# raynbowy23/RegT-GCN

Measured on NVIDIA B200. Metric: regt_gcn_fwd_bwd_samples_per_s, higher is better.
Workload: dtype f32 (3xTF32 on the tensor cores: fp32-equivalent, 1e-5 parity)

## Files before the change

### regt-gcn_b200/csrc/api.cu

```cuda
#include <stdlib.h>

#include "common.cuh"

namespace regt {

constexpr int F = REGT_F;

Route route_of(const regt_args* a) {
  const char* e = getenv("REGT_UNFUSED");
  const bool unfused = e && e[0] == '1';
  const bool tf32x3 = a->precision == REGT_PREC_TF32X3, bf16 = a->precision == REGT_PREC_BF16;
  const bool fused_step = a->fuse_head && a->y && a->d_out && a->loss;
  Route r{};
  r.cell = bf16 ? CellPath::Bf16
                : !tf32x3 ? CellPath::Fp32 : (!unfused && cell_f_fits(a)) ? CellPath::Tf32x3Fused : CellPath::Tf32x3Unfused;
  if (bf16 && fused_step && head_tc_fits(a->H, a->O))
    r.head = HeadPath::Bf16;
  else if (tf32x3 && a->H % 32 == 0 && head_f_fits(a->O) && (long long)a->B * a->N >= 128 && a->out)
    r.head = HeadPath::Tf32x3;
  else if (fused_step && head_fused_fits(a->H, a->O))
    r.head = HeadPath::FusedFfma;
  else
    r.head = HeadPath::Rows;
  r.g_tiled = r.cell == CellPath::Tf32x3Fused || r.cell == CellPath::Bf16;
  r.hid_partials = r.cell == CellPath::Bf16 && (r.head == HeadPath::Bf16 || r.head == HeadPath::FusedFfma);
  return r;
}

Layout make_layout(const regt_args* a, void* base) {
  Layout L{};
  L.route = route_of(a);
  Carver c(base);
  const size_t H = a->H, T = a->T, R = a->plan.R > 0 ? a->plan.R : 1, O = a->O;
  const size_t BN = (size_t)a->B * a->N, rows = BN * T;
  const size_t nseg = a->plan.nseg;
  L.Wzr = c.take<float>((F + H) * 2 * H);
  L.Wc = c.take<float>((F + H) * H);
  L.czr = c.take<float>(2 * H);
  L.cc = c.take<float>(H);
  L.M0t = c.take<float>(F * H);
  L.M1t = c.take<float>(R * F * H);
  L.c0 = c.take<float>(H);
  L.Lsum = c.take<float>(H * H);
  L.probs = c.take<float>(T);
  L.S = c.take<float>(BN * F * T);
  L.U = c.take<float>((size_t)a->B * (nseg ? nseg : 1) * F * T);
  if (L.route.cell == CellPath::Tf32x3Fused) {
    const size_t nqt = (BN + 127) / 128, rowsP = T * nqt * 128;
    const bool inf = a->inference != 0;
    L.tc_img_f = c.take<unsigned char>(F_IMG_BYTES);
    L.tc_img_b = c.take<unsigned char>(F_IMG_BYTES);
    L.Zp = c.take<float>(inf ? (size_t)TC_MAX_CTAS * 128 * H : rowsP * H);
    L.Rp = c.take<float>(inf ? 4 : rowsP * H);
    L.Hcp = c.take<float>(inf ? 4 : rowsP * H);
    L.Xt = c.take<float>(BN * F * T);
    L.h = c.take<float>(inf ? 4 : rowsP * H);
    L.hR = c.take<float>(inf ? 4 : rowsP * H);
    L.D = c.take<float>(inf ? 4 : rowsP * 4 * H);
    L.Feat = c.take<float>(inf ? 4 : nqt * 128 * 32);
    L.FeatT = c.take<float>(inf ? 4 : rowsP * 32);
    L.tc_dpp = c.take<float>(2 * (T * TC_MAX_CTAS + 64));
  } else if (L.route.cell != CellPath::Bf16) {
    L.h = c.take<float>(rows * H);
    L.Z = c.take<float>(rows * H);
    L.Rg = c.take<float>(rows * H);
    L.Hc = c.take<float>(rows * H);
    L.hR = c.take<float>(rows * H);
    L.Hn = c.take<float>(rows * H);
    L.D = c.take<float>(rows * 4 * H);
    L.Feat = c.take<float>(a->precision == REGT_PREC_TF32X3 ? rows * 32 : 4);
    L.bsplit = c.take<float>(a->precision == REGT_PREC_TF32X3 ? gemm_nt_scratch_floats((int)H, 2 * (int)H) : 4);
  } else {
    const size_t nqt = (BN + 127) / 128, plane = T * nqt * 128 * H;
    L.tc_img_f = c.take<unsigned char>(TC_IMG_BYTES);
    L.tc_img_b = c.take<unsigned char>(TC_IMG_BYTES);
    L.Zp = c.take<float>(plane);
    L.Rp = c.take<float>(plane);
    L.Hcp = c.take<float>(plane);
    L.dhp_p = c.take<float>(a->mode == REGT_MODE_REGIONAL ? plane : 4);
    L.Xt = c.take<float>(BN * F * T);
    L.hid_part = c.take<float>(T * nqt * 128 * H);
    L.tc_wpart = c.take<float>((size_t)TC_MAX_CTAS * 128 * 192);
    L.tc_dpp = c.take<float>(T * TC_MAX_CTAS + 64);
  }
  if (a->precision == REGT_PREC_TF32X3) {
    L.hf_rh = c.take<float>(BN * H);
    L.hf_do32 = c.take<float>(BN * 32);
    L.hf_split = c.take<float>(max(gemm_nt_scratch_floats(HEAD_HID, (int)H), gemm_nt_scratch_floats((int)H, HEAD_HID)));
    L.hf_loss_floats = BN / 8 + 2;
    L.hf_loss = c.take<float>(L.hf_loss_floats);
  }
  L.a1 = c.take<float>(BN * HEAD_HID);
  L.G = c.take<float>(((BN + 127) / 128) * 128 * H);
  L.d_a1 = c.take<float>(BN * HEAD_HID);
  L.dB = c.take<float>(3 * H * H);
  L.dP = c.take<float>(3 * H * F);
  L.dcg = c.take<float>(3 * H);
  L.dM0 = c.take<float>(H * F);
  L.dM1 = c.take<float>(R * H * F);
  L.dc0 = c.take<float>(H);
  L.dprobs = c.take<float>(T);
  size_t pf = (size_t)3 * WGRAD_SPLITS * H * H;
  pf = max(pf, (size_t)WGRAD_SPLITS * 4 * H * 32);
  pf = max(pf, (size_t)3 * H * H + 2 * 1024 * 64);
  pf = max(pf, (size_t)WGRAD_SPLITS * (3 * H * H + 4 * H * 32));
  pf = max(pf, (size_t)(2048 + R + 2) * H * F);
  pf = max(pf, (size_t)128 * T);
  pf = max(pf, (size_t)128 * (O * HEAD_HID + HEAD_HID * H));
  pf = max(pf, (size_t)152 * HEAD_HID * (H + 32));
  pf = max(pf, BN / 64 + 2);
  pf += H * HEAD_HID + HEAD_HID * O + 64;
  L.hpart = c.take<float>((size_t)148 * (HEAD_HID * H + O * HEAD_HID + HEAD_HID + O + 8));
  L.part = c.take<float>(pf);
  L.part_floats = pf;
  L.m1cp = c.take<int32_t>(R + 2);
  L.total = align_up(c.off, 256);
  return L;
}

static int validate(const regt_args* a, const char* who) {
  REGT_CHECK(a != nullptr, "%s: args is NULL", who);
  REGT_CHECK(a->B > 0 && a->N > 0 && a->T > 0 && a->O > 0, "%s: bad dims B=%d N=%d T=%d O=%d", who, a->B, a->N, a->T, a->O);
  REGT_CHECK(a->H >= 8 && a->H % 8 == 0 && a->H <= 1024, "%s: H=%d must be a multiple of 8 in [8,1024]", who, a->H);
  REGT_CHECK(a->mode >= 0 && a->mode <= 2, "%s: bad mode %d", who, a->mode);
  REGT_CHECK(a->x_rows == 0 || a->x_rows >= a->N, "%s: x_rows=%d must be 0 or >= N=%d", who, a->x_rows, a->N);
  REGT_CHECK(a->plan.N == a->N, "%s: plan built for %d nodes, args say %d", who, a->plan.N, a->N);
  REGT_CHECK((long long)a->B * a->N * a->T < (1ll << 31), "%s: B*N*T overflows int32 rows", who);
  REGT_CHECK(a->workspace && a->workspace_bytes >= regt_workspace_bytes(a), "%s: workspace missing or too small", who);
  REGT_CHECK(a->precision >= 0 && a->precision <= 2, "%s: bad precision %d", who, a->precision);
  return 0;
}

}

using namespace regt;

extern "C" size_t regt_workspace_bytes(const regt_args* a) {
  if (!a) return 0;
  return make_layout(a, nullptr).total;
}

extern "C" int regt_cell_forward(const regt_args* a) {
  if (validate(a, "regt_cell_forward")) return -1;
  REGT_CHECK(a->x && a->out_hidden, "regt_cell_forward: x / out_hidden is NULL");
  if (a->precision == REGT_PREC_TF32X3)
    REGT_CHECK(a->H % 32 == 0, "precision tf32x3 needs hidden %% 32 == 0 (got %d); use precision fp32", a->H);
  Layout L = make_layout(a, a->workspace);
  cudaStream_t st = (cudaStream_t)a->stream;
  prof_mark("<begin>", st);
  switch (L.route.cell) {
    case CellPath::Fp32: return cell_forward_fp32(a, L, st);
    case CellPath::Tf32x3Unfused: return cell_forward_g(a, L, st);
    case CellPath::Tf32x3Fused: return cell_forward_f(a, L, st);
    case CellPath::Bf16: return cell_forward_tc(a, L, st);
  }
  return -1;
}

extern "C" int regt_cell_backward(const regt_args* a) {
  if (validate(a, "regt_cell_backward")) return -1;
  REGT_CHECK(!a->inference, "regt_cell_backward: the forward ran with inference=1 (no activations were saved)");
  if (a->precision == REGT_PREC_TF32X3)
    REGT_CHECK(a->H % 32 == 0, "precision tf32x3 needs hidden %% 32 == 0 (got %d); use precision fp32", a->H);
  Layout L = make_layout(a, a->workspace);
  cudaStream_t st = (cudaStream_t)a->stream;
  prof_mark("<begin>", st);
  switch (L.route.cell) {
    case CellPath::Fp32: return cell_backward_fp32(a, L, st);
    case CellPath::Tf32x3Unfused: return cell_backward_g(a, L, st);
    case CellPath::Tf32x3Fused: return cell_backward_f(a, L, st);
    case CellPath::Bf16: return cell_backward_tc(a, L, st);
  }
  return -1;
}

static int validate_x(const regt_args* a, const regt_xgrad_plan* xp, const char* who) {
  REGT_CHECK(a != nullptr, "%s: args is NULL", who);
  REGT_CHECK(a->precision != REGT_PREC_BF16, "%s: precision bf16 keeps no gate-gradient plane; use fp32 or tf32x3", who);
  REGT_CHECK(a->x_rows == 0 || a->x_rows == a->N,
             "%s: region shards (x_rows=%d != N=%d) are not supported: their halo rows belong to other ranks", who, a->x_rows, a->N);
  REGT_CHECK(!a->inference, "%s: the forward ran with inference=1 (no activations were saved)", who);
  if (validate(a, who)) return -1;
  REGT_CHECK(xp && xp->N == a->N && xp->n_src == 2 * a->N + a->plan.nseg && xp->rowptr && xp->col && xp->val,
             "%s: transposed plan missing or built for another graph", who);
  return 0;
}

extern "C" size_t regt_cell_backward_x_scratch_bytes(const regt_args* a, const regt_xgrad_plan* xp) {
  if (!a || !xp) return 0;
  return cell_backward_x_scratch_bytes(a, xp);
}

extern "C" int regt_cell_backward_x(const regt_args* a, const regt_xgrad_plan* xp, float* d_x, void* scratch,
                                    size_t scratch_bytes) {
  if (validate_x(a, xp, "regt_cell_backward_x")) return -1;
  REGT_CHECK(d_x, "regt_cell_backward_x: d_x is NULL");
  REGT_CHECK(scratch && scratch_bytes >= cell_backward_x_scratch_bytes(a, xp), "regt_cell_backward_x: scratch missing or too small");
  if (a->precision == REGT_PREC_TF32X3)
    REGT_CHECK(a->H % 32 == 0, "precision tf32x3 needs hidden %% 32 == 0 (got %d); use precision fp32", a->H);
  Layout L = make_layout(a, a->workspace);
  cudaStream_t st = (cudaStream_t)a->stream;
  prof_mark("<begin>", st);
  return cell_backward_x(a, L, xp, d_x, scratch, st);
}

extern "C" int regt_head_forward(const regt_args* a) {
  if (validate(a, "regt_head_forward")) return -1;
  REGT_CHECK(a->out_hidden && a->out, "regt_head_forward: out_hidden / out is NULL");
  Layout L = make_layout(a, a->workspace);
  prof_mark("<begin>", (cudaStream_t)a->stream);
  return head_forward(a, L, (cudaStream_t)a->stream);
}

extern "C" int regt_head_backward(const regt_args* a) {
  if (validate(a, "regt_head_backward")) return -1;
  REGT_CHECK(!a->inference, "regt_head_backward: the forward ran with inference=1 (no activations were saved)");
  Layout L = make_layout(a, a->workspace);
  prof_mark("<begin>", (cudaStream_t)a->stream);
  return head_backward(a, L, (cudaStream_t)a->stream);
}

extern "C" int regt_debug_route(const regt_args* a, int32_t* out) {
  REGT_CHECK(a && out, "regt_debug_route: args and out must be non-NULL");
  const Route r = route_of(a);
  out[0] = (int32_t)r.cell;
  out[1] = (int32_t)r.head;
  out[2] = r.g_tiled;
  out[3] = r.hid_partials;
  return 0;
}
```

### regt-gcn_b200/csrc/common.cuh

```cuda
#pragma once
#include <cuda_runtime.h>
#include <stdint.h>
#include <stdio.h>

#include "regt_b200.h"

namespace regt {

void set_error(const char* fmt, ...);
void count_launch(int n = 1);
void prof_mark(const char* name, cudaStream_t st);
cudaStream_t fork_side(cudaStream_t main);
int join_side(cudaStream_t main);

#define REGT_CHECK(cond, ...)         \
  do {                                \
    if (!(cond)) {                    \
      regt::set_error(__VA_ARGS__);   \
      return -1;                      \
    }                                 \
  } while (0)

#define REGT_CUDA(expr)                                                                  \
  do {                                                                                   \
    cudaError_t _e = (expr);                                                             \
    if (_e != cudaSuccess) {                                                             \
      regt::set_error("%s failed: %s (%s:%d)", #expr, cudaGetErrorString(_e), __FILE__, __LINE__); \
      return -2;                                                                         \
    }                                                                                    \
  } while (0)

#define REGT_LAUNCH_CHECK()                                                              \
  do {                                                                                   \
    regt::count_launch();                                                                \
    cudaError_t _e = cudaGetLastError();                                                 \
    if (_e != cudaSuccess) {                                                             \
      regt::set_error("kernel launch failed: %s (%s:%d)", cudaGetErrorString(_e), __FILE__, __LINE__); \
      return -3;                                                                         \
    }                                                                                    \
  } while (0)

#define REGT_LAUNCHED(name, st)       \
  do {                                \
    REGT_LAUNCH_CHECK();              \
    regt::prof_mark(name, st);        \
  } while (0)

inline size_t align_up(size_t v, size_t a) { return (v + a - 1) / a * a; }
inline int cdiv(long long a, long long b) { return (int)((a + b - 1) / b); }

struct Carver {
  char* base;
  size_t off;
  explicit Carver(void* p) : base((char*)p), off(0) {}
  template <typename T>
  T* take(size_t n) {
    off = align_up(off, 256);
    T* r = base ? (T*)(base + off) : (T*)nullptr;
    off += n * sizeof(T);
    return r;
  }
};

__device__ __forceinline__ float sigmoidf_(float v) { return 1.0f / (1.0f + expf(-v)); }

__device__ __forceinline__ size_t g_off(long long q, int n, int H, int tiled) {
  return tiled ? ((((size_t)(q >> 7) * (H >> 2) + (n >> 2)) * 128 + (size_t)(q & 127)) * 4 + (n & 3)) : ((size_t)q * H + n);
}

inline int sm_count() {
  static int n = 0;
  if (n == 0) {
    int dev = 0;
    if (cudaGetDevice(&dev) != cudaSuccess || cudaDeviceGetAttribute(&n, cudaDevAttrMultiProcessorCount, dev) != cudaSuccess || n <= 0) n = 148;
  }
  return n;
}

enum class CellPath { Fp32, Tf32x3Unfused, Tf32x3Fused, Bf16 };
enum class HeadPath { Rows, FusedFfma, Tf32x3, Bf16 };
struct Route {
  CellPath cell;
  HeadPath head;
  bool g_tiled;
  bool hid_partials;
};
Route route_of(const regt_args* a);
bool cell_f_fits(const regt_args* a);
bool head_fused_fits(int H, int O);
bool head_tc_fits(int H, int O);
bool head_f_fits(int O);

struct Layout {
  Route route;
  float* Wzr;
  float* Wc;
  float* czr;
  float* cc;
  float* M0t;
  float* M1t;
  float* c0;
  float* Lsum;
  float* probs;
  float* S;
  float* U;
  float* h;
  float* Z;
  float* Rg;
  float* Hc;
  float* hR;
  float* Hn;
  float* a1;
  float* G;
  float* d_a1;
  float* D;
  float* Feat;
  float* hf_rh;
  float* hf_do32;
  float* hf_split;
  float* hf_loss;
  size_t hf_loss_floats;
  float* FeatT;
  float* bsplit;
  float* dB;
  float* dP;
  float* dcg;
  float* dM0;
  float* dM1;
  float* dc0;
  float* dprobs;
  float* hpart;
  float* part;
  size_t part_floats;
  int32_t* m1cp;
  unsigned char* tc_img_f;
  unsigned char* tc_img_b;
  float *Zp, *Rp, *Hcp, *dhp_p;
  float* Xt;
  float* hid_part;
  float* tc_wpart;
  float* tc_dpp;
  size_t total;
};
constexpr int TC_MAX_CTAS = 160;
constexpr int TC_IMG_BYTES = 160 * 1024;
constexpr int F_IMG_BYTES = 432 * 1024;

Layout make_layout(const regt_args* a, void* base);

constexpr int HEAD_HID = 128;
constexpr int WGRAD_SPLITS = 64;

int cell_forward_fp32(const regt_args* a, const Layout& L, cudaStream_t st);
int cell_backward_fp32(const regt_args* a, const Layout& L, cudaStream_t st);
int cell_forward_g(const regt_args* a, const Layout& L, cudaStream_t st);
int cell_backward_g(const regt_args* a, const Layout& L, cudaStream_t st);
int cell_forward_f(const regt_args* a, const Layout& L, cudaStream_t st);
int cell_backward_f(const regt_args* a, const Layout& L, cudaStream_t st);
int cell_forward_tc(const regt_args* a, const Layout& L, cudaStream_t st);
int cell_backward_tc(const regt_args* a, const Layout& L, cudaStream_t st);
size_t cell_backward_x_scratch_bytes(const regt_args* a, const regt_xgrad_plan* xp);
int cell_backward_x(const regt_args* a, const Layout& L, const regt_xgrad_plan* xp, float* d_x, void* scratch, cudaStream_t st);
int head_forward(const regt_args* a, const Layout& L, cudaStream_t st);
int head_backward(const regt_args* a, const Layout& L, cudaStream_t st);
int head_forward_f(const regt_args* a, const Layout& L, cudaStream_t st);
int head_backward_f(const regt_args* a, const Layout& L, cudaStream_t st);
int head_forward_tc(const regt_args* a, const Layout& L, cudaStream_t st);

int launch_prep(const regt_args* a, const Layout& L, cudaStream_t st);
int launch_chain(const regt_args* a, const Layout& L, cudaStream_t st);
int launch_spmm_rows(const int32_t* rowptr, const int32_t* col, const float* val, const float* x, float* y, int B,
                     int n_out, int n_in, int width, cudaStream_t st);
int launch_feat_tc(const regt_graph_plan& p, const float* x, int B, int xN, int T, float* Xt, float* St, float* Ut, cudaStream_t st);
struct TNBatch;
int launch_wgrad_tn(const TNBatch& batch, long long rows, int splits, cudaStream_t st);
int launch_reduce_splits(const float* part, float* out, long long count, int splits, int accumulate, cudaStream_t st);
int launch_colsum(const float* A, int lda, int C, long long rows, int splits, float* part, cudaStream_t st);
int launch_wgrad_m1(const regt_args* a, const Layout& L, cudaStream_t st);
int launch_wgrad_m1_kt(const regt_args* a, const Layout& L, cudaStream_t st);
int launch_f_sum_dpp(const double* part, int nparts, int T, float* dprobs, cudaStream_t st);
int launch_fw_scatter(const float* Cp, int splits, int H, const Layout& L, cudaStream_t st);
size_t gemm_nt_scratch_floats(int N, int K);
int launch_gemm_nt_tma(const float* A, long long lda, const float* Bt, long long ldb, float* C, long long ldc, long long M, int N,
                       int K, float* scratch, cudaStream_t st);
int launch_gemm_tn(const float* A, long long lda, const float* B, long long ldb, float* Cp, long long M, int K, int N, int splits,
                   cudaStream_t st, const float* B2, long long ldb2, float* Cp2, long long c2_split, int relu_b);
int launch_gemm_tn_tma(const float* A, long long lda, long long M, int Ktot, int nseg, const int* seg_k0, const int* seg_b,
                       float* const* seg_C, const float* const* Bs, const long long* ldbs, int N, int splits, const float* B2,
                       long long ldb2, float* C2, long long c2_split, cudaStream_t st, int relu_b);
int launch_gemm_kt(const float* AT, long long ntile, int Ktot, int nseg, const int* seg_k0, const int* seg_k1, const int* seg_b,
                   float* const* seg_C, const float* const* BTs, int N, int splits, const float* FT, float* C2, long long c2_split,
                   cudaStream_t st);
int head_part_stride_host(int H, int O);
int launch_head_grad_reduce(const regt_args* a, const Layout& L, cudaStream_t st);
int launch_head_dw1_tf32x3(const regt_args* a, const Layout& L, const float* ones, cudaStream_t st);
int head_tc_grid(const regt_args* a);
int tc_num_chunks(const regt_args* a);

}
```

### regt-gcn_b200/csrc/gemm_tma.cu

```cuda
#include <cuda.h>

#include "cell_tc.cuh"

namespace regt {
using namespace tc;

namespace {
constexpr int KC = 32;
constexpr int TILE = 128 * 128;
constexpr int MAXS = 6;
constexpr int SMEM_BUDGET = 227 * 1024 - 1024;

__device__ __forceinline__ uint32_t tf32_rn(float a) {
  uint32_t u;
  asm("cvt.rna.tf32.f32 %0, %1;" : "=r"(u) : "f"(a));
  return u;
}
__device__ __forceinline__ void split4(const float4 v, float4& hi, float4& lo) {
  hi.x = __uint_as_float(tf32_rn(v.x)); hi.y = __uint_as_float(tf32_rn(v.y));
  hi.z = __uint_as_float(tf32_rn(v.z)); hi.w = __uint_as_float(tf32_rn(v.w));
  lo.x = v.x - hi.x; lo.y = v.y - hi.y; lo.z = v.z - hi.z; lo.w = v.w - hi.w;
}
__device__ __forceinline__ void tma_2d(void* dst, const CUtensorMap* map, int c0, int c1, uint64_t* bar) {
  asm volatile(
      "cp.async.bulk.tensor.2d.shared::cluster.global.tile.mbarrier::complete_tx::bytes [%0], [%1, {%2, %3}], [%4];" ::"r"(
          smem_u32(dst)),
      "l"(reinterpret_cast<uint64_t>(map)), "r"(c0), "r"(c1), "r"(smem_u32(bar))
      : "memory");
}
__device__ __forceinline__ void tmap_prefetch(const CUtensorMap* map) {
  asm volatile("prefetch.tensormap [%0];" ::"l"(reinterpret_cast<uint64_t>(map)) : "memory");
}

typedef CUresult (*EncodeFn)(CUtensorMap*, CUtensorMapDataType, cuuint32_t, void*, const cuuint64_t*, const cuuint64_t*,
                             const cuuint32_t*, const cuuint32_t*, CUtensorMapInterleave, CUtensorMapSwizzle,
                             CUtensorMapL2promotion, CUtensorMapFloatOOBfill);
EncodeFn encoder() {
  static EncodeFn fn = nullptr;
  if (!fn) {
    void* p = nullptr;
    cudaDriverEntryPointQueryResult q;
    if (cudaGetDriverEntryPoint("cuTensorMapEncodeTiled", &p, cudaEnableDefault, &q) == cudaSuccess && q == cudaDriverEntryPointSuccess)
      fn = (EncodeFn)p;
  }
  return fn;
}
int tmap_2d(CUtensorMap* m, const float* base, long long cols, long long rows, long long ld, int box_rows, const char* who) {
  EncodeFn enc = encoder();
  REGT_CHECK(enc != nullptr, "%s: cuTensorMapEncodeTiled is not available from this driver", who);
  REGT_CHECK(((uintptr_t)base % 16 == 0) && ld % 4 == 0, "%s: TMA operands need 16-byte aligned base and pitch", who);
  cuuint64_t dims[2] = {(cuuint64_t)cols, (cuuint64_t)rows};
  cuuint64_t strides[1] = {(cuuint64_t)ld * 4};
  cuuint32_t box[2] = {32, (cuuint32_t)box_rows};
  cuuint32_t estr[2] = {1, 1};
  const CUresult r = enc(m, CU_TENSOR_MAP_DATA_TYPE_FLOAT32, 2, (void*)base, dims, strides, box, estr, CU_TENSOR_MAP_INTERLEAVE_NONE,
                         CU_TENSOR_MAP_SWIZZLE_128B, CU_TENSOR_MAP_L2_PROMOTION_L2_256B, CU_TENSOR_MAP_FLOAT_OOB_FILL_NONE);
  REGT_CHECK(r == CUDA_SUCCESS, "%s: cuTensorMapEncodeTiled failed (%d) cols=%lld rows=%lld ld=%lld", who, (int)r, cols, rows, ld);
  return 0;
}

__global__ void k_split_hilo(const float* __restrict__ B, long long ldb, int N, int K, int Np, int Kp, float* __restrict__ hi,
                             float* __restrict__ lo) {
  const long long i = blockIdx.x * (long long)blockDim.x + threadIdx.x;
  if (i >= (long long)Np * Kp) return;
  const int n = (int)(i / Kp), k = (int)(i - (long long)n * Kp);
  const float v = (n < N && k < K) ? __ldg(B + (size_t)n * ldb + k) : 0.f;
  const float h = __uint_as_float(tf32_rn(v));
  hi[i] = h;
  lo[i] = v - h;
}

struct NtArgs {
  CUtensorMap ta, tbh, tbl;
  float* C;
  long long M, ldc;
  int N, K;
  int resident;
  int ns;
};
constexpr int NT_CONV = 256;
constexpr int NT_W_TMA = NT_CONV / 32;
constexpr int NT_W_MMA = NT_W_TMA + 1;
constexpr int NT_W_EPI = NT_W_MMA + 1;
constexpr int NT_THREADS = (NT_W_EPI + 4) * 32;

constexpr int TS_SLOTS = 4;
__global__ void __launch_bounds__(NT_THREADS, 1) k_gemm_nt_tma_ts(const __grid_constant__ NtArgs a) {
  extern __shared__ __align__(1024) uint8_t smem_raw[];
  uint8_t* sm = smem_raw + ((1024u - (smem_u32(smem_raw) & 1023u)) & 1023u);
  __shared__ uint64_t bar_tma[MAXS], bar_rfree[MAXS], bar_afull[TS_SLOTS], bar_afree[TS_SLOTS], bar_b, bar_acc_full[2], bar_acc_free[2];
  __shared__ uint32_t tmem_base_s;
  const int tid = threadIdx.x, warp = tid >> 5, lane = tid & 31;
  const int ns = a.ns;
  const int nchunks = (a.K + KC - 1) / KC;
  const int ntn = (a.N + 127) / 128;
  const long long ntiles = ((a.M + 127) / 128) * ntn;
  const int stage_bytes = a.resident ? TILE : 3 * TILE;
  uint8_t* bres = sm;
  uint8_t* stages = sm + (a.resident ? nchunks * 2 * TILE : 0);
  if (tid == 0) {
    for (int s = 0; s < ns; ++s) {
      mbar_init(&bar_tma[s], 1);
      mbar_init(&bar_rfree[s], a.resident ? NT_CONV : NT_CONV + 1);
    }
    for (int s = 0; s < TS_SLOTS; ++s) {
      mbar_init(&bar_afull[s], NT_CONV);
      mbar_init(&bar_afree[s], 1);
    }
    mbar_init(&bar_b, 1);
    for (int b = 0; b < 2; ++b) {
      mbar_init(&bar_acc_full[b], 1);
      mbar_init(&bar_acc_free[b], 128);
    }
    fence_barrier_init();
  }
  if (warp == NT_W_MMA) tmem_alloc(&tmem_base_s, 512);
  tc_fence_before();
  __syncthreads();
  tc_fence_after();
  const uint32_t tmem = tmem_base_s;
  const uint32_t tmem_a = tmem + 256;

  if (warp < NT_W_TMA) {
    const int q = warp & 3, half = warp >> 2;
    const int r = q * 32 + lane;
    const uint32_t tl = tmem_a + ((uint32_t)(q * 32) << 16) + 16 * half;
    long long gc = 0;
    for (long long tile = blockIdx.x; tile < ntiles; tile += gridDim.x) {
      for (int kc = 0; kc < nchunks; ++kc, ++gc) {
        const int s = (int)(gc % ns), sl = (int)(gc % TS_SLOTS);
        mbar_wait(&bar_tma[s], (uint32_t)((gc / ns) & 1));
        const uint8_t* rw = stages + (size_t)s * stage_bytes + r * 128;
        uint32_t hi[16], lo[16];
#pragma unroll
        for (int c = 0; c < 4; ++c) {
          const float4 v = *reinterpret_cast<const float4*>(rw + (((half * 4 + c) ^ (r & 7)) << 4));
          float4 h, l;
          split4(v, h, l);
          hi[4 * c] = __float_as_uint(h.x); hi[4 * c + 1] = __float_as_uint(h.y); hi[4 * c + 2] = __float_as_uint(h.z); hi[4 * c + 3] = __float_as_uint(h.w);
          lo[4 * c] = __float_as_uint(l.x); lo[4 * c + 1] = __float_as_uint(l.y); lo[4 * c + 2] = __float_as_uint(l.z); lo[4 * c + 3] = __float_as_uint(l.w);
        }
        if ((hi[0] | hi[4] | hi[8] | hi[12]) == 0x7FC0DEADu) __nanosleep(1);
        mbar_arrive(&bar_rfree[s]);
        if (gc >= TS_SLOTS) {
          mbar_wait(&bar_afree[sl], (uint32_t)((gc / TS_SLOTS - 1) & 1));
          tc_fence_after();
        }
        tmem_st16(tl + 64 * sl, hi);
        tmem_st16(tl + 64 * sl + 32, lo);
        tmem_st_wait();
        tc_fence_before();
        mbar_arrive(&bar_afull[sl]);
      }
    }
  } else if (warp == NT_W_TMA) {
    if (lane == 0) {
      tmap_prefetch(&a.ta);
      tmap_prefetch(&a.tbh);
      tmap_prefetch(&a.tbl);
      if (a.resident) {
        mbar_arrive_expect_tx(&bar_b, (uint32_t)(nchunks * 2 * TILE));
        for (int kc = 0; kc < nchunks; ++kc) {
          tma_2d(bres + (size_t)kc * 2 * TILE, &a.tbh, kc * KC, 0, &bar_b);
          tma_2d(bres + (size_t)kc * 2 * TILE + TILE, &a.tbl, kc * KC, 0, &bar_b);
        }
      }
      long long gc = 0;
      for (long long tile = blockIdx.x; tile < ntiles; tile += gridDim.x) {
        const int m0 = (int)((tile / ntn) * 128), n0 = (int)(tile % ntn) * 128;
        for (int kc = 0; kc < nchunks; ++kc, ++gc) {
          const int s = (int)(gc % ns);
          if (gc >= ns) mbar_wait(&bar_rfree[s], (uint32_t)((gc / ns - 1) & 1));
          uint8_t* st = stages + (size_t)s * stage_bytes;
          mbar_arrive_expect_tx(&bar_tma[s], (uint32_t)stage_bytes);
          tma_2d(st, &a.ta, kc * KC, m0, &bar_tma[s]);
          if (!a.resident) {
            tma_2d(st + TILE, &a.tbh, kc * KC, n0, &bar_tma[s]);
            tma_2d(st + 2 * TILE, &a.tbl, kc * KC, n0, &bar_tma[s]);
          }
        }
      }
    }
  } else if (warp == NT_W_MMA) {
    const uint32_t bres0 = smem_u32(bres), stage0 = smem_u32(stages);
    if (a.resident) mbar_wait(&bar_b, 0);
    long long gc = 0, li = 0;
    for (long long tile = blockIdx.x; tile < ntiles; tile += gridDim.x, ++li) {
      const int nt = min(128, a.N - (int)(tile % ntn) * 128);
      const uint32_t idesc = make_idesc(FMT_TF32, 128, nt, 0, 0);
      const int buf = (int)(li & 1);
      if (li >= 2) {
        mbar_wait(&bar_acc_free[buf], (uint32_t)((li / 2 - 1) & 1));
        tc_fence_after();
      }
      for (int kc = 0; kc < nchunks; ++kc, ++gc) {
        const int sl = (int)(gc % TS_SLOTS);
        mbar_wait(&bar_afull[sl], (uint32_t)((gc / TS_SLOTS) & 1));
        tc_fence_after();
        if (lane == 0) {
          const uint32_t ah = tmem_a + 64 * sl, al = ah + 32;
          const int s = (int)(gc % ns);
          const uint32_t bt = a.resident ? bres0 + kc * 2 * TILE : stage0 + s * stage_bytes + TILE;
#pragma unroll
          for (int p = 0; p < 3; ++p) {
            const uint32_t ap = (p == 1) ? al : ah, bp = bt + (p == 2 ? TILE : 0);
#pragma unroll
            for (int k = 0; k < KC / 8; ++k)
              umma_ts_tf32(tmem + buf * 128, ap + 8 * k, make_desc(bp + k * 32, 16, 1024, LAYOUT_SW128), idesc,
                           (kc > 0 || p > 0 || k > 0) ? 1u : 0u);
          }
          umma_commit(&bar_afree[sl]);
          if (!a.resident) umma_commit(&bar_rfree[s]);
          if (kc + 1 == nchunks) umma_commit(&bar_acc_full[buf]);
        }
        __syncwarp();
      }
    }
    tc_fence_before();
  } else {
    const int r = (warp & 3) * 32 + lane;
    const uint32_t tlane = tmem + ((uint32_t)((warp & 3) * 32) << 16);
    long long li = 0;
    for (long long tile = blockIdx.x; tile < ntiles; tile += gridDim.x, ++li) {
      const int buf = (int)(li & 1);
      const int n0 = (int)(tile % ntn) * 128;
      const int nt = min(128, a.N - n0);
      const long long arow = (tile / ntn) * 128 + r;
      const bool a_ok = arow < a.M;
      float* cp = a.C + (a_ok ? arow : 0) * a.ldc + n0;
      mbar_wait(&bar_acc_full[buf], (uint32_t)((li / 2) & 1));
      tc_fence_after();
      for (int c0 = 0; c0 < nt; c0 += 32) {
        float v[32];
        if (c0 + 32 <= nt) {
          tmem_ld32(tlane + buf * 128 + c0, v);
        } else {
          float u[16];
          tmem_ld16(tlane + buf * 128 + c0, u);
#pragma unroll
          for (int j = 0; j < 16; ++j) v[j] = u[j];
        }
        if (a_ok) {
          const int w = min(32, nt - c0);
#pragma unroll
          for (int j = 0; j < 32; j += 4)
            if (j < w) *reinterpret_cast<float4*>(cp + c0 + j) = make_float4(v[j], v[j + 1], v[j + 2], v[j + 3]);
        }
      }
      tc_fence_before();
      mbar_arrive(&bar_acc_free[buf]);
    }
  }
  __syncthreads();
  if (warp == NT_W_MMA) tmem_dealloc(tmem, 512);
}

struct TnSeg {
  int k0, k1;
  int b;
  float* C;
};
struct TnArgs {
  CUtensorMap ta, tb[2], tf;
  TnSeg seg[4];
  int nseg;
  float* C2;
  long long c2_split;
  long long M, chunk;
  int N, N2;
  int relu_b;
};
constexpr int TN_CONV = 256;
constexpr int TN_W_MMA = TN_CONV / 32;
constexpr int TN_W_TMA = TN_W_MMA + 1;
constexpr int TN_THREADS = (TN_W_TMA + 1) * 32;
constexpr int TN_NR = 2, TN_NC = 2;
constexpr int TN_BOX = 32 * 128;
constexpr int TN_RAW = 9 * TN_BOX;
constexpr int TN_BT = (128 + 32) * 128;
constexpr int TN_CV = 2 * TILE + 2 * TN_BT;
constexpr int TN_GROUP = 8;
constexpr int TN_ACC = 256;
static_assert(TN_NR * TN_RAW + TN_NC * TN_CV <= SMEM_BUDGET, "gemm_tn stages exceed shared memory");

__global__ void __launch_bounds__(TN_THREADS, 1) k_gemm_tn_tma(const __grid_constant__ TnArgs a) {
  extern __shared__ __align__(1024) uint8_t smem_raw[];
  uint8_t* sm = smem_raw + ((1024u - (smem_u32(smem_raw) & 1023u)) & 1023u);
  __shared__ uint64_t bar_raw[TN_NR], bar_rfree[TN_NR], bar_full[TN_NC], bar_empty[TN_NC], bar_done, bar_acc_free[2];
  __shared__ uint32_t tmem_base_s;
  const int tid = threadIdx.x, warp = tid >> 5, lane = tid & 31;
  const int kg = blockIdx.x * 128;
  int si = 0;
  for (int s = 1; s < a.nseg; ++s)
    if (kg >= a.seg[s].k0) si = s;
  const int sk0 = a.seg[si].k0, sk1 = a.seg[si].k1, sb = a.seg[si].b;
  float* segC = a.seg[si].C;
  const int n0 = blockIdx.y * 128;
  const int kt = min(128, sk1 - kg);
  const int nt = sb >= 0 ? max(0, min(128, a.N - n0)) : 0;
  const int n2 = (blockIdx.y == 0) ? a.N2 : 0;
  const int ntot = nt + n2;
  const long long r0 = (long long)blockIdx.z * a.chunk, r1 = min(a.M, r0 + a.chunk);
  const int nchunks = ntot > 0 ? (int)max(0ll, (r1 - r0 + KC - 1) / KC) : 0;
  uint8_t* raw = sm;
  uint8_t* cv = sm + TN_NR * TN_RAW;
  if (tid == 0) {
    for (int s = 0; s < TN_NR; ++s) {
      mbar_init(&bar_raw[s], 1);
      mbar_init(&bar_rfree[s], TN_CONV);
    }
    for (int s = 0; s < TN_NC; ++s) {
      mbar_init(&bar_full[s], TN_CONV);
      mbar_init(&bar_empty[s], 1);
    }
    mbar_init(&bar_done, 1);
    mbar_init(&bar_acc_free[0], TN_CONV);
    mbar_init(&bar_acc_free[1], TN_CONV);
    fence_barrier_init();
  }
  if (warp == TN_W_MMA) tmem_alloc(&tmem_base_s, 512);
  tc_fence_before();
  __syncthreads();
  tc_fence_after();
  const uint32_t tmem = tmem_base_s;
  const int ablk = kt / 32, bblk = (nt + 31) / 32;

  if (warp < TN_W_MMA) {
    const int blk = warp & 3, half = warp >> 2;
    const bool a_ok = blk < ablk, b_ok = blk < bblk;
    const int orow = (warp & 3) * 32 + lane;
    const uint32_t tlane = tmem + ((uint32_t)((warp & 3) * 32) << 16);
    float acc[5][16];
#pragma unroll
    for (int i = 0; i < 5; ++i)
#pragma unroll
      for (int j = 0; j < 16; ++j) acc[i][j] = 0.f;
    int drained = 0;
    auto drain = [&](int buf) {
      tc_fence_after();
#pragma unroll
      for (int i = 0; i < 5; ++i) {
        const int c0 = half * 16 + 32 * i;
        if (c0 < ntot) {
          float v[16];
          tmem_ld16(tlane + buf * TN_ACC + c0, v);
#pragma unroll
          for (int j = 0; j < 16; ++j) acc[i][j] += v[j];
        }
      }
      tc_fence_before();
      mbar_arrive(&bar_acc_free[buf]);
    };
    for (int kc = 0; kc < nchunks; ++kc) {
      const int rs = kc % TN_NR, cs = kc % TN_NC;
      mbar_wait(&bar_raw[rs], (uint32_t)((kc / TN_NR) & 1));
      const uint8_t* rw = raw + rs * TN_RAW;
      float4 av[4], bv[4], fv = make_float4(0.f, 0.f, 0.f, 0.f);
#pragma unroll
      for (int c = 0; c < 4; ++c) {
        const uint32_t off = (uint32_t)(lane * 128 + (((half * 4 + c) ^ (lane & 7)) << 4));
        av[c] = a_ok ? *reinterpret_cast<const float4*>(rw + blk * TN_BOX + off) : make_float4(0.f, 0.f, 0.f, 0.f);
        bv[c] = b_ok ? *reinterpret_cast<const float4*>(rw + (4 + blk) * TN_BOX + off) : make_float4(0.f, 0.f, 0.f, 0.f);
      }
      if (a.relu_b) {
#pragma unroll
        for (int c = 0; c < 4; ++c) bv[c] = make_float4(fmaxf(bv[c].x, 0.f), fmaxf(bv[c].y, 0.f), fmaxf(bv[c].z, 0.f), fmaxf(bv[c].w, 0.f));
      }
      if (n2) fv = *reinterpret_cast<const float4*>(rw + 8 * TN_BOX + lane * 128 + ((warp ^ (lane & 7)) << 4));
      {
        const uint32_t dep = __float_as_uint(av[0].x) | __float_as_uint(av[1].x) | __float_as_uint(av[2].x) | __float_as_uint(av[3].x) |
                             __float_as_uint(bv[0].x) | __float_as_uint(bv[1].x) | __float_as_uint(bv[2].x) | __float_as_uint(bv[3].x) |
                             __float_as_uint(fv.x);
        if (dep == 0x7FC0DEADu) __nanosleep(1);
        mbar_arrive(&bar_rfree[rs]);
      }
      if (kc >= TN_NC) mbar_wait(&bar_empty[cs], (uint32_t)((kc / TN_NC - 1) & 1));
      if (kc >= TN_GROUP + TN_NC - 1 && (kc - (TN_NC - 1)) % TN_GROUP == 0) {
        drain(drained & 1);
        ++drained;
      }
      uint8_t* st = cv + cs * TN_CV;
#pragma unroll
      for (int c = 0; c < 4; ++c) {
        float4 hi, lo;
        split4(av[c], hi, lo);
        const float ah[4] = {hi.x, hi.y, hi.z, hi.w}, al[4] = {lo.x, lo.y, lo.z, lo.w};
        split4(bv[c], hi, lo);
        const float bh[4] = {hi.x, hi.y, hi.z, hi.w}, bl[4] = {lo.x, lo.y, lo.z, lo.w};
#pragma unroll
        for (int e = 0; e < 4; ++e) {
          const int col = blk * 32 + 16 * half + 4 * c + e;
          const uint32_t off = sw128_off(col, lane * 4, 128);
          *reinterpret_cast<float*>(st + off) = ah[e];
          *reinterpret_cast<float*>(st + TILE + off) = al[e];
          if (col < nt) {
            *reinterpret_cast<float*>(st + 2 * TILE + off) = bh[e];
            *reinterpret_cast<float*>(st + 2 * TILE + TN_BT + off) = bl[e];
          }
        }
      }
      if (n2) {
        float4 hi, lo;
        split4(fv, hi, lo);
        const float fh[4] = {hi.x, hi.y, hi.z, hi.w}, fl[4] = {lo.x, lo.y, lo.z, lo.w};
#pragma unroll
        for (int e = 0; e < 4; ++e) {
          const uint32_t off = sw128_off(nt + 4 * warp + e, lane * 4, 128);
          *reinterpret_cast<float*>(st + 2 * TILE + off) = fh[e];
          *reinterpret_cast<float*>(st + 2 * TILE + TN_BT + off) = fl[e];
        }
      }
      fence_proxy_async();
      mbar_arrive(&bar_full[cs]);
    }
    const int ngroups = (nchunks + TN_GROUP - 1) / TN_GROUP;
    if (nchunks > 0) mbar_wait(&bar_done, 0);
    for (; drained < ngroups; ++drained) drain(drained & 1);
    const bool row_ok = orow < kt;
    float* cp = nt > 0 ? segC + ((size_t)blockIdx.z * (sk1 - sk0) + (kg - sk0) + (row_ok ? orow : 0)) * a.N + n0 : nullptr;
    float* cp2 = n2 ? a.C2 + (size_t)blockIdx.z * a.c2_split + (size_t)(kg + (row_ok ? orow : 0)) * 32 : nullptr;
#pragma unroll
    for (int i = 0; i < 5; ++i) {
      const int c0 = half * 16 + 32 * i;
      if (c0 < ntot && row_ok) {
        float* o = c0 < nt ? cp + c0 : cp2 + (c0 - nt);
#pragma unroll
        for (int j = 0; j < 16; j += 4) *reinterpret_cast<float4*>(o + j) = make_float4(acc[i][j], acc[i][j + 1], acc[i][j + 2], acc[i][j + 3]);
      }
    }
  } else if (warp == TN_W_MMA) {
    const uint32_t idesc = make_idesc(FMT_TF32, 128, max(ntot, 16), 0, 0);
    const uint32_t base = smem_u32(cv);
    for (int kc = 0; kc < nchunks; ++kc) {
      const int s = kc % TN_NC;
      const int g = kc / TN_GROUP, buf = g & 1, kg0 = kc % TN_GROUP;
      if (kg0 == 0 && g >= 2) {
        mbar_wait(&bar_acc_free[buf], (uint32_t)((g / 2 - 1) & 1));
        tc_fence_after();
      }
      mbar_wait(&bar_full[s], (uint32_t)((kc / TN_NC) & 1));
      tc_fence_after();
      if (lane == 0) {
        const uint32_t st = base + s * TN_CV;
#pragma unroll
        for (int p = 0; p < 3; ++p) {
          const uint32_t at = st + (p == 1 ? TILE : 0), bt = st + 2 * TILE + (p == 2 ? TN_BT : 0);
#pragma unroll
          for (int k = 0; k < KC / 8; ++k)
            umma<FMT_TF32>(tmem + buf * TN_ACC, make_desc(at + k * 32, 16, 1024, LAYOUT_SW128), make_desc(bt + k * 32, 16, 1024, LAYOUT_SW128),
                           idesc, (kg0 > 0 || p > 0 || k > 0) ? 1u : 0u);
        }
        umma_commit(&bar_empty[s]);
        if (kc + 1 == nchunks) umma_commit(&bar_done);
      }
      __syncwarp();
    }
    tc_fence_before();
  } else {
    if (lane == 0 && nchunks > 0) {
      tmap_prefetch(&a.ta);
      if (sb >= 0) tmap_prefetch(&a.tb[sb]);
      if (n2) tmap_prefetch(&a.tf);
      const uint32_t bytes = (uint32_t)((ablk + bblk + (n2 ? 1 : 0)) * TN_BOX);
      for (int kc = 0; kc < nchunks; ++kc) {
        const int rs = kc % TN_NR;
        if (kc >= TN_NR) mbar_wait(&bar_rfree[rs], (uint32_t)((kc / TN_NR - 1) & 1));
        uint8_t* rw = raw + rs * TN_RAW;
        const int row = (int)(r0 + (long long)kc * KC);
        mbar_arrive_expect_tx(&bar_raw[rs], bytes);
        for (int b = 0; b < ablk; ++b) tma_2d(rw + b * TN_BOX, &a.ta, kg + b * 32, row, &bar_raw[rs]);
        for (int b = 0; b < bblk; ++b) tma_2d(rw + (4 + b) * TN_BOX, &a.tb[sb], n0 + b * 32, row, &bar_raw[rs]);
        if (n2) tma_2d(rw + 8 * TN_BOX, &a.tf, 0, row, &bar_raw[rs]);
      }
    }
  }
  __syncthreads();
  if (warp == TN_W_MMA) tmem_dealloc(tmem, 512);
}

struct KtArgs {
  CUtensorMap ta, tb[2], tf;
  TnSeg seg[4];
  int nseg;
  float* C2;
  long long c2_split;
  long long ntile, tiles_per_split;
  int Ktot, N, N2;
};
constexpr int KT_RAW = 2 * TILE + TN_BOX;

__global__ void __launch_bounds__(TN_THREADS, 1) k_gemm_kt(const __grid_constant__ KtArgs a) {
  extern __shared__ __align__(1024) uint8_t smem_raw[];
  uint8_t* sm = smem_raw + ((1024u - (smem_u32(smem_raw) & 1023u)) & 1023u);
  __shared__ uint64_t bar_raw[TN_NR], bar_rfree[TN_NR], bar_full[TN_NC], bar_empty[TN_NC], bar_done, bar_acc_free[2];
  __shared__ uint32_t tmem_base_s;
  const int tid = threadIdx.x, warp = tid >> 5, lane = tid & 31;
  const int kg = blockIdx.x * 128;
  int si = 0;
  for (int s = 1; s < a.nseg; ++s)
    if (kg >= a.seg[s].k0) si = s;
  const int sk0 = a.seg[si].k0, sk1 = a.seg[si].k1, sb = a.seg[si].b;
  float* segC = a.seg[si].C;
  const int kt = min(128, sk1 - kg);
  const int kt2 = min(128, a.Ktot - kg);
  const int nt = sb >= 0 ? a.N : 0;
  const int n2 = a.N2;
  const int ntot = nt + n2;
  const long long t0 = (long long)blockIdx.z * a.tiles_per_split, t1 = min(a.ntile, t0 + a.tiles_per_split);
  const int nchunks = ntot > 0 ? (int)max(0ll, (t1 - t0) * 4) : 0;
  uint8_t* raw = sm;
  uint8_t* cv = sm + TN_NR * KT_RAW;
  if (tid == 0) {
    for (int s = 0; s < TN_NR; ++s) {
      mbar_init(&bar_raw[s], 1);
      mbar_init(&bar_rfree[s], TN_CONV);
    }
    for (int s = 0; s < TN_NC; ++s) {
      mbar_init(&bar_full[s], TN_CONV);
      mbar_init(&bar_empty[s], 1);
    }
    mbar_init(&bar_done, 1);
    mbar_init(&bar_acc_free[0], TN_CONV);
    mbar_init(&bar_acc_free[1], TN_CONV);
    fence_barrier_init();
  }
  if (warp == TN_W_MMA) tmem_alloc(&tmem_base_s, 512);
  tc_fence_before();
  __syncthreads();
  tc_fence_after();
  const uint32_t tmem = tmem_base_s;

  if (warp < TN_W_MMA) {
    const int row = (warp & 3) * 32 + lane, half = warp >> 2;
    const int frow = tid >> 3, fpc = tid & 7;
    const bool b_ok = row < nt;
    const int orow = row;
    const uint32_t tlane = tmem + ((uint32_t)((warp & 3) * 32) << 16);
    float acc[5][16];
#pragma unroll
    for (int i = 0; i < 5; ++i)
#pragma unroll
      for (int j = 0; j < 16; ++j) acc[i][j] = 0.f;
    int drained = 0;
    auto drain = [&](int buf) {
      tc_fence_after();
#pragma unroll
      for (int i = 0; i < 5; ++i) {
        const int c0 = half * 16 + 32 * i;
        if (c0 < ntot) {
          float v[16];
          tmem_ld16(tlane + buf * TN_ACC + c0, v);
#pragma unroll
          for (int j = 0; j < 16; ++j) acc[i][j] += v[j];
        }
      }
      tc_fence_before();
      mbar_arrive(&bar_acc_free[buf]);
    };
    uint32_t offs[4];
#pragma unroll
    for (int c = 0; c < 4; ++c) offs[c] = (uint32_t)(row * 128 + (((half * 4 + c) ^ (row & 7)) << 4));
    const uint32_t foff = (uint32_t)(frow * 128 + ((fpc ^ (frow & 7)) << 4));
    for (int kc = 0; kc < nchunks; ++kc) {
      const int rs = kc % TN_NR, cs = kc % TN_NC;
      mbar_wait(&bar_raw[rs], (uint32_t)((kc / TN_NR) & 1));
      const uint8_t* rw = raw + rs * KT_RAW;
      float4 av[4], bv[4], fv = make_float4(0.f, 0.f, 0.f, 0.f);
#pragma unroll
      for (int c = 0; c < 4; ++c) {
        av[c] = *reinterpret_cast<const float4*>(rw + offs[c]);
        bv[c] = b_ok ? *reinterpret_cast<const float4*>(rw + TILE + offs[c]) : make_float4(0.f, 0.f, 0.f, 0.f);
      }
      if (n2) fv = *reinterpret_cast<const float4*>(rw + 2 * TILE + foff);
      {
        const uint32_t dep = __float_as_uint(av[0].x) | __float_as_uint(av[1].x) | __float_as_uint(av[2].x) | __float_as_uint(av[3].x) |
                             __float_as_uint(bv[0].x) | __float_as_uint(bv[1].x) | __float_as_uint(bv[2].x) | __float_as_uint(bv[3].x) |
                             __float_as_uint(fv.x);
        if (dep == 0x7FC0DEADu) __nanosleep(1);
        mbar_arrive(&bar_rfree[rs]);
      }
      if (kc >= TN_NC) mbar_wait(&bar_empty[cs], (uint32_t)((kc / TN_NC - 1) & 1));
      if (kc >= TN_GROUP + TN_NC - 1 && (kc - (TN_NC - 1)) % TN_GROUP == 0) {
        drain(drained & 1);
        ++drained;
      }
      uint8_t* st = cv + cs * TN_CV;
#pragma unroll
      for (int c = 0; c < 4; ++c) {
        float4 hi, lo;
        split4(av[c], hi, lo);
        *reinterpret_cast<float4*>(st + offs[c]) = hi;
        *reinterpret_cast<float4*>(st + TILE + offs[c]) = lo;
        if (b_ok) {
          split4(bv[c], hi, lo);
          *reinterpret_cast<float4*>(st + 2 * TILE + offs[c]) = hi;
          *reinterpret_cast<float4*>(st + 2 * TILE + TN_BT + offs[c]) = lo;
        }
      }
      if (n2) {
        float4 hi, lo;
        split4(fv, hi, lo);
        *reinterpret_cast<float4*>(st + 2 * TILE + nt * 128 + foff) = hi;
        *reinterpret_cast<float4*>(st + 2 * TILE + TN_BT + nt * 128 + foff) = lo;
      }
      fence_proxy_async();
      mbar_arrive(&bar_full[cs]);
    }
    const int ngroups = (nchunks + TN_GROUP - 1) / TN_GROUP;
    if (nchunks > 0) mbar_wait(&bar_done, 0);
    for (; drained < ngroups; ++drained) drain(drained & 1);
    const bool row_ok = orow < kt, row_ok2 = orow < kt2;
    float* cp = nt > 0 ? segC + ((size_t)blockIdx.z * (sk1 - sk0) + (kg - sk0) + (row_ok ? orow : 0)) * a.N : nullptr;
    float* cp2 = n2 ? a.C2 + (size_t)blockIdx.z * a.c2_split + (size_t)(kg + (row_ok2 ? orow : 0)) * 32 : nullptr;
#pragma unroll
    for (int i = 0; i < 5; ++i) {
      const int c0 = half * 16 + 32 * i;
      if (c0 < ntot && (c0 < nt ? row_ok : row_ok2)) {
        float* o = c0 < nt ? cp + c0 : cp2 + (c0 - nt);
#pragma unroll
        for (int j = 0; j < 16; j += 4) *reinterpret_cast<float4*>(o + j) = make_float4(acc[i][j], acc[i][j + 1], acc[i][j + 2], acc[i][j + 3]);
      }
    }
  } else if (warp == TN_W_MMA) {
    const uint32_t idesc = make_idesc(FMT_TF32, 128, max(ntot, 16), 0, 0);
    const uint32_t base = smem_u32(cv);
    for (int kc = 0; kc < nchunks; ++kc) {
      const int s = kc % TN_NC;
      const int g = kc / TN_GROUP, buf = g & 1, kg0 = kc % TN_GROUP;
      if (kg0 == 0 && g >= 2) {
        mbar_wait(&bar_acc_free[buf], (uint32_t)((g / 2 - 1) & 1));
        tc_fence_after();
      }
      mbar_wait(&bar_full[s], (uint32_t)((kc / TN_NC) & 1));
      tc_fence_after();
      if (lane == 0) {
        const uint32_t st = base + s * TN_CV;
#pragma unroll
        for (int p = 0; p < 3; ++p) {
          const uint32_t at = st + (p == 1 ? TILE : 0), bt = st + 2 * TILE + (p == 2 ? TN_BT : 0);
#pragma unroll
          for (int k = 0; k < KC / 8; ++k)
            umma<FMT_TF32>(tmem + buf * TN_ACC, make_desc(at + k * 32, 16, 1024, LAYOUT_SW128), make_desc(bt + k * 32, 16, 1024, LAYOUT_SW128),
                           idesc, (kg0 > 0 || p > 0 || k > 0) ? 1u : 0u);
        }
        umma_commit(&bar_empty[s]);
        if (kc + 1 == nchunks) umma_commit(&bar_done);
      }
      __syncwarp();
    }
    tc_fence_before();
  } else {
    if (lane == 0 && nchunks > 0) {
      tmap_prefetch(&a.ta);
      if (sb >= 0) tmap_prefetch(&a.tb[sb]);
      if (n2) tmap_prefetch(&a.tf);
      const uint32_t bytes = (uint32_t)(TILE + (sb >= 0 ? a.N * 128 : 0) + (n2 ? TN_BOX : 0));
      for (int kc = 0; kc < nchunks; ++kc) {
        const int rs = kc % TN_NR;
        if (kc >= TN_NR) mbar_wait(&bar_rfree[rs], (uint32_t)((kc / TN_NR - 1) & 1));
        uint8_t* rw = raw + rs * KT_RAW;
        const long long tile = t0 + kc / 4;
        const int k0 = (kc & 3) * KC;
        mbar_arrive_expect_tx(&bar_raw[rs], bytes);
        const long long tq = tile * 4 + (k0 >> 5);
        tma_2d(rw, &a.ta, 0, (int)(tq * a.Ktot + kg), &bar_raw[rs]);
        if (sb >= 0) tma_2d(rw + TILE, &a.tb[sb], 0, (int)(tq * a.N), &bar_raw[rs]);
        if (n2) tma_2d(rw + 2 * TILE, &a.tf, 0, (int)(tq * 32), &bar_raw[rs]);
      }
    }
  }
  __syncthreads();
  if (warp == TN_W_MMA) tmem_dealloc(tmem, 512);
}
}

size_t gemm_nt_scratch_floats(int N, int K) { return (size_t)2 * ((N + 127) / 128 * 128) * ((K + KC - 1) / KC * KC); }

int launch_gemm_nt_tma(const float* A, long long lda, const float* Bt, long long ldb, float* C, long long ldc, long long M, int N,
                       int K, float* scratch, cudaStream_t st) {
  REGT_CHECK(A && Bt && C && scratch && M >= 1 && N > 0 && N % 16 == 0 && K > 0 && K % 4 == 0 && ldc % 4 == 0 &&
                 ((uintptr_t)C % 16) == 0 && ((uintptr_t)scratch % 16) == 0,
             "gemm_nt_tma: bad operands (M=%lld N=%d K=%d)", M, N, K);
  const int Np = (N + 127) / 128 * 128, Kp = (K + KC - 1) / KC * KC, nchunks = Kp / KC;
  float* hi = scratch;
  float* lo = scratch + (size_t)Np * Kp;
  k_split_hilo<<<cdiv((long long)Np * Kp, 256), 256, 0, st>>>(Bt, ldb, N, K, Np, Kp, hi, lo);
  REGT_LAUNCHED("k_split_hilo", st);
  NtArgs a{};
  if (tmap_2d(&a.ta, A, K, M, lda, 128, "gemm_nt_tma(A)")) return -1;
  if (tmap_2d(&a.tbh, hi, Kp, Np, Kp, 128, "gemm_nt_tma(B hi)")) return -1;
  if (tmap_2d(&a.tbl, lo, Kp, Np, Kp, 128, "gemm_nt_tma(B lo)")) return -1;
  a.C = C; a.M = M; a.ldc = ldc; a.N = N; a.K = K;
  a.resident = (N <= 128 && nchunks * 2 * TILE + 2 * 2 * TILE <= SMEM_BUDGET) ? 1 : 0;
  const int fixed = a.resident ? nchunks * 2 * TILE : 0;
  const int stage_ts = a.resident ? TILE : 3 * TILE;
  a.ns = min(MAXS, (SMEM_BUDGET - fixed) / stage_ts);
  const long long ntiles = (long long)cdiv(M, 128) * cdiv(N, 128);
  const size_t smem_ts = (size_t)fixed + (size_t)a.ns * stage_ts + 1024;
  REGT_CUDA(cudaFuncSetAttribute(k_gemm_nt_tma_ts, cudaFuncAttributeMaxDynamicSharedMemorySize, (int)smem_ts));
  k_gemm_nt_tma_ts<<<(int)min(ntiles, (long long)sm_count()), NT_THREADS, smem_ts, st>>>(a);
  REGT_LAUNCHED("k_gemm_nt_tma_ts", st);
  return 0;
}

int launch_gemm_tn_tma(const float* A, long long lda, long long M, int Ktot, int nseg, const int* seg_k0, const int* seg_b,
                       float* const* seg_C, const float* const* Bs, const long long* ldbs, int N, int splits, const float* B2,
                       long long ldb2, float* C2, long long c2_split, cudaStream_t st, int relu_b) {
  REGT_CHECK(A && nseg >= 1 && nseg <= 4 && Ktot % 32 == 0 && N % 32 == 0 && splits > 0 && M >= 1, "gemm_tn_tma: bad shape");
  REGT_CHECK(!B2 || (C2 && ldb2 % 4 == 0), "gemm_tn_tma: bad second operand");
  TnArgs a{};
  if (tmap_2d(&a.ta, A, Ktot, M, lda, 32, "gemm_tn_tma(A)")) return -1;
  bool any_b = false;
  for (int s = 0; s < nseg; ++s) {
    a.seg[s].k0 = seg_k0[s];
    a.seg[s].k1 = s + 1 < nseg ? seg_k0[s + 1] : Ktot;
    a.seg[s].b = seg_b[s];
    a.seg[s].C = seg_C[s];
    REGT_CHECK(nseg == 1 || a.seg[s].k0 % 128 == 0, "gemm_tn_tma: segment boundaries must be multiples of 128");
    REGT_CHECK(seg_b[s] < 2 && (seg_b[s] < 0 || (seg_C[s] && Bs[seg_b[s]])), "gemm_tn_tma: segment %d has no operand / output", s);
    any_b |= seg_b[s] >= 0;
  }
  for (int b = 0; b < 2; ++b) {
    bool used = false;
    for (int s = 0; s < nseg; ++s) used |= seg_b[s] == b;
    if (used && tmap_2d(&a.tb[b], Bs[b], N, M, ldbs[b], 32, "gemm_tn_tma(B)")) return -1;
  }
  REGT_CHECK(any_b || B2, "gemm_tn_tma: nothing to contract with");
  if (B2 && tmap_2d(&a.tf, B2, 32, M, ldb2, 32, "gemm_tn_tma(B2)")) return -1;
  a.nseg = nseg;
  a.C2 = C2;
  a.c2_split = c2_split > 0 ? c2_split : (long long)Ktot * 32;
  a.M = M;
  long long chunk = (M + splits - 1) / splits;
  a.chunk = (chunk + KC - 1) / KC * KC;
  a.N = any_b ? N : 0;
  a.N2 = B2 ? 32 : 0;
  a.relu_b = relu_b;
  const size_t smem = (size_t)TN_NR * TN_RAW + (size_t)TN_NC * TN_CV + 1024;
  REGT_CUDA(cudaFuncSetAttribute(k_gemm_tn_tma, cudaFuncAttributeMaxDynamicSharedMemorySize, (int)smem));
  k_gemm_tn_tma<<<dim3(cdiv(Ktot, 128), max(1, cdiv(a.N, 128)), splits), TN_THREADS, smem, st>>>(a);
  REGT_LAUNCHED("k_gemm_tn_tma", st);
  return 0;
}

int launch_gemm_kt(const float* AT, long long ntile, int Ktot, int nseg, const int* seg_k0, const int* seg_k1, const int* seg_b,
                   float* const* seg_C, const float* const* BTs, int N, int splits, const float* FT, float* C2, long long c2_split,
                   cudaStream_t st) {
  REGT_CHECK(AT && nseg >= 1 && nseg <= 4 && Ktot % 128 == 0 && N % 8 == 0 && N >= 16 && N <= 128 && splits > 0 && ntile > 0 && FT && C2,
             "gemm_kt: bad shape (Ktot=%d N=%d)", Ktot, N);
  REGT_CHECK(ntile * 4 * Ktot < (1ll << 31), "gemm_kt: tile count overflows the TMA coordinate");
  KtArgs a{};
  if (tmap_2d(&a.ta, AT, 32, ntile * 4 * Ktot, 32, 128, "gemm_kt(A^T)")) return -1;
  for (int s = 0; s < nseg; ++s) {
    a.seg[s].k0 = seg_k0[s];
    a.seg[s].k1 = seg_k1[s];
    a.seg[s].b = seg_b[s];
    a.seg[s].C = seg_C[s];
    REGT_CHECK(a.seg[s].k0 % 128 == 0, "gemm_kt: segment starts must be multiples of 128");
    REGT_CHECK(seg_b[s] < 2 && (seg_b[s] < 0 || (seg_C[s] && BTs[seg_b[s]])), "gemm_kt: segment %d has no operand / output", s);
  }
  for (int b = 0; b < 2; ++b) {
    bool used = false;
    for (int s = 0; s < nseg; ++s) used |= seg_b[s] == b;
    if (used && tmap_2d(&a.tb[b], BTs[b], 32, ntile * 4 * N, 32, N, "gemm_kt(B^T)")) return -1;
  }
  if (tmap_2d(&a.tf, FT, 32, ntile * 4 * 32, 32, 32, "gemm_kt(F^T)")) return -1;
  a.nseg = nseg;
  a.C2 = C2;
  a.c2_split = c2_split > 0 ? c2_split : (long long)Ktot * 32;
  a.ntile = ntile;
  a.tiles_per_split = (ntile + splits - 1) / splits;
  a.Ktot = Ktot; a.N = N; a.N2 = 32;
  const size_t smem = (size_t)TN_NR * KT_RAW + (size_t)TN_NC * TN_CV + 1024;
  REGT_CUDA(cudaFuncSetAttribute(k_gemm_kt, cudaFuncAttributeMaxDynamicSharedMemorySize, (int)smem));
  k_gemm_kt<<<dim3(Ktot / 128, 1, splits), TN_THREADS, smem, st>>>(a);
  REGT_LAUNCHED("k_gemm_kt", st);
  return 0;
}

int launch_gemm_tn(const float* A, long long lda, const float* B, long long ldb, float* Cp, long long M, int K, int N, int splits,
                   cudaStream_t st, const float* B2, long long ldb2, float* Cp2, long long c2_split, int relu_b) {
  const int k0 = 0, sb = N > 0 ? 0 : -1;
  float* cs[1] = {Cp};
  const float* bs[2] = {B, nullptr};
  const long long lds[2] = {ldb, 0};
  return launch_gemm_tn_tma(A, lda, M, K, 1, &k0, &sb, cs, bs, lds, N, splits, B2, ldb2, Cp2, c2_split, st, relu_b);
}

}

extern "C" int regt_debug_gemm_nt_tma(const float* A, int64_t lda, const float* Bt, int64_t ldb, float* C, int64_t ldc, int64_t M,
                                      int32_t N, int32_t K, float* scratch, regt_stream_t stream) {
  return regt::launch_gemm_nt_tma(A, lda, Bt, ldb, C, ldc, M, N, K, scratch, (cudaStream_t)stream);
}
extern "C" int regt_debug_gemm_tn_tma(const float* A, int64_t lda, const float* B, int64_t ldb, float* Cp, int64_t M, int32_t K,
                                      int32_t N, int32_t splits, const float* B2, int64_t ldb2, float* Cp2, regt_stream_t stream) {
  return regt::launch_gemm_tn(A, lda, B, ldb, Cp, M, K, N, splits, (cudaStream_t)stream, B2, ldb2, Cp2, 0, 0);
}
extern "C" int regt_debug_gemm_tn_multi(const float* A, int64_t lda, int64_t M, int32_t H, const float* B0, const float* B1,
                                        float* C0, float* C1, int32_t splits, const float* B2, float* C2, regt_stream_t stream) {
  const int k0[3] = {0, 2 * H, 3 * H}, sb[3] = {0, 1, -1};
  float* cs[3] = {C0, C1, nullptr};
  const float* bs[2] = {B0, B1};
  const long long lds[2] = {H, H};
  return regt::launch_gemm_tn_tma(A, lda, M, 4 * H, 3, k0, sb, cs, bs, lds, H, splits, B2, 32, C2, 0, (cudaStream_t)stream, 0);
}
extern "C" int regt_debug_gemm_kt(const float* AT, int64_t ntile, int32_t H, const float* B0T, const float* B1T, const float* FT,
                                  float* C0, float* C1, float* C2, int32_t splits, regt_stream_t stream) {
  int k0[3], k1[3], sb[3], ns;
  float* cs[3];
  if (H == 128) {
    ns = 3;
    k0[0] = 0; k1[0] = 256; sb[0] = 0; cs[0] = C0;
    k0[1] = 256; k1[1] = 384; sb[1] = 1; cs[1] = C1;
    k0[2] = 384; k1[2] = 512; sb[2] = -1; cs[2] = nullptr;
  } else {
    ns = 2;
    k0[0] = 0; k1[0] = 128; sb[0] = 0; cs[0] = C0;
    k0[1] = 128; k1[1] = 192; sb[1] = 1; cs[1] = C1;
  }
  const float* bs[2] = {B0T, B1T};
  return regt::launch_gemm_kt(AT, ntile, 4 * H, ns, k0, k1, sb, cs, bs, H, splits, FT, C2, 0, (cudaStream_t)stream);
}
```

### regt-gcn_b200/csrc/head_f.cu

```cuda
#include "common.cuh"

namespace regt {

namespace {
__global__ void __launch_bounds__(256) k_hf_relu(const float4* __restrict__ hid, float4* __restrict__ rh, long long n4) {
  const long long i = blockIdx.x * (long long)blockDim.x + threadIdx.x;
  if (i >= n4) return;
  const float4 v = __ldg(hid + i);
  rh[i] = make_float4(fmaxf(v.x, 0.f), fmaxf(v.y, 0.f), fmaxf(v.z, 0.f), fmaxf(v.w, 0.f));
}

constexpr int HF_O = 16;
__global__ void __launch_bounds__(256) k_hf_mid(float* __restrict__ a1, const float* __restrict__ b1, const float* __restrict__ w2,
                                                const float* __restrict__ b2, const float* __restrict__ y, long long BN, int O, float scale,
                                                float* __restrict__ out, float* __restrict__ d_out, float* __restrict__ loss_part) {
  __shared__ float red[8];
  const int lane = threadIdx.x & 31, warp = threadIdx.x >> 5;
  float w[HF_O][4];
#pragma unroll
  for (int o = 0; o < HF_O; ++o) {
    const float4 t = o < O ? __ldg(reinterpret_cast<const float4*>(w2 + (size_t)o * HEAD_HID) + lane) : make_float4(0.f, 0.f, 0.f, 0.f);
    w[o][0] = t.x; w[o][1] = t.y; w[o][2] = t.z; w[o][3] = t.w;
  }
  const float4 bb = __ldg(reinterpret_cast<const float4*>(b1) + lane);
  float lsum = 0.f;
  for (long long q = blockIdx.x * 8ll + warp; q < BN; q += (long long)gridDim.x * 8) {
    const float4 p = reinterpret_cast<const float4*>(a1 + q * HEAD_HID)[lane];
    const float a[4] = {fmaxf(p.x + bb.x, 0.f), fmaxf(p.y + bb.y, 0.f), fmaxf(p.z + bb.z, 0.f), fmaxf(p.w + bb.w, 0.f)};
    reinterpret_cast<float4*>(a1 + q * HEAD_HID)[lane] = make_float4(a[0], a[1], a[2], a[3]);
    float s16[HF_O];
#pragma unroll
    for (int o = 0; o < HF_O; ++o) {
      float s = a[0] * w[o][0];
      s = fmaf(a[1], w[o][1], s); s = fmaf(a[2], w[o][2], s); s = fmaf(a[3], w[o][3], s);
      s16[o] = s;
    }
    float s8[8], s4[4], s2[2];
    {
      const bool up = lane & 16;
#pragma unroll
      for (int i = 0; i < 8; ++i) {
        const float keep = up ? s16[i + 8] : s16[i], send = up ? s16[i] : s16[i + 8];
        s8[i] = keep + __shfl_xor_sync(0xffffffffu, send, 16);
      }
    }
    {
      const bool up = lane & 8;
#pragma unroll
      for (int i = 0; i < 4; ++i) {
        const float keep = up ? s8[i + 4] : s8[i], send = up ? s8[i] : s8[i + 4];
        s4[i] = keep + __shfl_xor_sync(0xffffffffu, send, 8);
      }
    }
    {
      const bool up = lane & 4;
#pragma unroll
      for (int i = 0; i < 2; ++i) {
        const float keep = up ? s4[i + 2] : s4[i], send = up ? s4[i] : s4[i + 2];
        s2[i] = keep + __shfl_xor_sync(0xffffffffu, send, 4);
      }
    }
    float mine;
    {
      const bool up = lane & 2;
      const float keep = up ? s2[1] : s2[0], send = up ? s2[0] : s2[1];
      mine = keep + __shfl_xor_sync(0xffffffffu, send, 2);
    }
    mine += __shfl_xor_sync(0xffffffffu, mine, 1);
    const int o = lane >> 1;
    if ((lane & 1) == 0 && o < O) {
      const float v = mine + __ldg(b2 + o);
      out[q * O + o] = v;
      if (y) {
        const float diff = v - __ldg(y + q * O + o);
        lsum = fmaf(diff, diff, lsum);
        d_out[q * O + o] = 2.0f * diff * scale;
      }
    }
  }
  if (y) {
#pragma unroll
    for (int d = 16; d > 0; d >>= 1) lsum += __shfl_xor_sync(0xffffffffu, lsum, d);
    if (lane == 0) red[warp] = lsum;
    __syncthreads();
    if (threadIdx.x == 0) {
      float s = 0.f;
#pragma unroll
      for (int i = 0; i < 8; ++i) s += red[i];
      loss_part[blockIdx.x] = s * scale;
    }
  }
}

__global__ void __launch_bounds__(256) k_hf_da1(const float* __restrict__ a1, const float* __restrict__ w2, const float* __restrict__ d_out,
                                                long long BN, int O, float* __restrict__ d_a1, float* __restrict__ dO32) {
  const int lane = threadIdx.x & 31, warp = threadIdx.x >> 5;
  const long long q = blockIdx.x * 8ll + warp;
  if (q >= BN) return;
  const float dv = lane < O ? __ldg(d_out + q * O + lane) : 0.f;
  float acc[4] = {0.f, 0.f, 0.f, 0.f};
#pragma unroll
  for (int o = 0; o < HF_O; ++o) {
    if (o < O) {
      const float d = __shfl_sync(0xffffffffu, dv, o);
      const float4 t = __ldg(reinterpret_cast<const float4*>(w2 + (size_t)o * HEAD_HID) + lane);
      acc[0] = fmaf(d, t.x, acc[0]); acc[1] = fmaf(d, t.y, acc[1]); acc[2] = fmaf(d, t.z, acc[2]); acc[3] = fmaf(d, t.w, acc[3]);
    }
  }
  const float4 a = __ldg(reinterpret_cast<const float4*>(a1 + q * HEAD_HID) + lane);
  reinterpret_cast<float4*>(d_a1 + q * HEAD_HID)[lane] =
      make_float4(a.x > 0.f ? acc[0] : 0.f, a.y > 0.f ? acc[1] : 0.f, a.z > 0.f ? acc[2] : 0.f, a.w > 0.f ? acc[3] : 0.f);
  dO32[q * 32 + lane] = lane < O ? dv : (lane == 16 ? 1.0f : 0.f);
}

__global__ void __launch_bounds__(256) k_hf_gmask(const float4* __restrict__ gpre, const float4* __restrict__ hid, const float4* __restrict__ dh,
                                                  long long BN, int H, int tiled, float* __restrict__ G) {
  const long long i = blockIdx.x * (long long)blockDim.x + threadIdx.x;
  const int h4 = H >> 2;
  if (i >= BN * h4) return;
  const long long q = i / h4;
  const int n = (int)(i - q * h4) * 4;
  const float4 g = __ldg(gpre + i), h = __ldg(hid + i);
  float4 v = make_float4(h.x > 0.f ? g.x : 0.f, h.y > 0.f ? g.y : 0.f, h.z > 0.f ? g.z : 0.f, h.w > 0.f ? g.w : 0.f);
  if (dh) {
    const float4 d = __ldg(dh + i);
    v.x += d.x; v.y += d.y; v.z += d.z; v.w += d.w;
  }
  *reinterpret_cast<float4*>(G + g_off(q, n, H, tiled)) = v;
}
__global__ void k_hf_w1t(const float* __restrict__ w1, int H, float* __restrict__ W1t) {
  const int i = blockIdx.x * blockDim.x + threadIdx.x;
  if (i >= H * HEAD_HID) return;
  const int k = i / HEAD_HID, m = i % HEAD_HID;
  W1t[i] = w1[(size_t)m * H + k];
}
__global__ void k_hf_dw2(const float* __restrict__ C2, int splits, int O, int acc, float* __restrict__ dW2) {
  const int i = blockIdx.x * blockDim.x + threadIdx.x;
  if (i >= O * HEAD_HID || !dW2) return;
  const int o = i / HEAD_HID, n = i % HEAD_HID;
  float s = 0.f;
  for (int z = 0; z < splits; ++z) s += C2[((size_t)z * HEAD_HID + n) * 32 + o];
  dW2[i] = acc ? dW2[i] + s : s;
}
}

bool head_f_fits(int O) { return O <= HF_O; }

int head_forward_f(const regt_args* a, const Layout& L, cudaStream_t st) {
  const int H = a->H, O = a->O;
  const long long BN = (long long)a->B * a->N;
  const int Nl = a->loss_nodes > 0 ? a->loss_nodes : a->N;
  k_hf_relu<<<cdiv(BN * H / 4, 256), 256, 0, st>>>(reinterpret_cast<const float4*>(a->out_hidden), reinterpret_cast<float4*>(L.hf_rh), BN * H / 4);
  REGT_LAUNCHED("k_hf_relu", st);
  if (launch_gemm_nt_tma(L.hf_rh, H, a->p.head_w1, H, L.a1, HEAD_HID, BN, HEAD_HID, H, L.hf_split, st)) return -1;
  const int nblk = (int)min((long long)cdiv(BN, 8), 1184ll);
  REGT_CHECK(!a->y || (a->loss && a->d_out), "head_forward: y given but loss/d_out is NULL");
  REGT_CHECK(!a->y || (size_t)nblk <= L.hf_loss_floats, "head_forward: loss partial buffer too small");
  k_hf_mid<<<nblk, 256, 0, st>>>(L.a1, a->p.head_b1, a->p.head_w2, a->p.head_b2, a->y, BN, O, 1.0f / ((float)Nl * (float)O), a->out,
                                 a->d_out, L.hf_loss);
  REGT_LAUNCHED("k_hf_mid", st);
  if (a->y) return launch_reduce_splits(L.hf_loss, a->loss, 1, nblk, 0, st);
  return 0;
}

int head_backward_f(const regt_args* a, const Layout& L, cudaStream_t st) {
  const int H = a->H, O = a->O;
  const long long BN = (long long)a->B * a->N;
  k_hf_da1<<<cdiv(BN, 8), 256, 0, st>>>(L.a1, a->p.head_w2, a->d_out, BN, O, L.d_a1, L.hf_do32);
  REGT_LAUNCHED("k_hf_da1", st);
  float* W1t = L.part + L.part_floats - (size_t)H * HEAD_HID;
  k_hf_w1t<<<cdiv((long long)H * HEAD_HID, 256), 256, 0, st>>>(a->p.head_w1, H, W1t);
  REGT_LAUNCHED("k_hf_w1t", st);
  if (launch_gemm_nt_tma(L.d_a1, HEAD_HID, W1t, HEAD_HID, L.hf_rh, H, BN, H, HEAD_HID, L.hf_split, st)) return -1;
  k_hf_gmask<<<cdiv(BN * (H / 4), 256), 256, 0, st>>>(reinterpret_cast<const float4*>(L.hf_rh), reinterpret_cast<const float4*>(a->out_hidden),
                                                      reinterpret_cast<const float4*>(a->d_hidden), BN, H, L.route.g_tiled, L.G);
  REGT_LAUNCHED("k_hf_gmask", st);
  float* part = L.part;
  if (launch_head_dw1_tf32x3(a, L, L.hf_do32, st)) return -1;
  const int s2 = (int)max(1ll, min(148ll, BN / 256));
  float* p3 = part;
  if (launch_gemm_tn(L.a1, HEAD_HID, nullptr, 0, nullptr, BN, HEAD_HID, 0, s2, st, L.hf_do32, 32, p3, 0, 0)) return -1;
  k_hf_dw2<<<cdiv(O * HEAD_HID, 256), 256, 0, st>>>(p3, s2, O, a->accumulate, a->g.head_w2);
  REGT_LAUNCHED("k_hf_dw2", st);
  const int s3 = (int)max(1ll, min(128ll, BN / 128));
  if (launch_colsum(a->d_out, O, O, BN, s3, part, st)) return -1;
  return launch_reduce_splits(part, a->g.head_b2, O, s3, a->accumulate, st);
}

}
```

Measured before the change: 230.2.

## Fuse head ReLU, mid-layer and grad mask into TF32x3 GEMM epilogues

Turns the TMEM GEMM kernel into a template with a pluggable epilogue functor and an optional ReLU applied to A while it is split into TF32 hi/lo parts. The head forward now fuses ReLU, the first-layer GEMM, bias, second layer, output, loss and d_out into one kernel. The backward grad-mask is fused into the dA GEMM epilogue. This drops the hf_rh intermediate buffer and several elementwise launches with their HBM round-trips, at the cost of heavier epilogue work on the four epilogue warps and more template instantiations.

```diff
diff --git a/regt-gcn_b200/csrc/api.cu b/regt-gcn_b200/csrc/api.cu
--- a/regt-gcn_b200/csrc/api.cu
+++ b/regt-gcn_b200/csrc/api.cu
@@ -84,10 +84,9 @@
     L.tc_dpp = c.take<float>(T * TC_MAX_CTAS + 64);
   }
   if (a->precision == REGT_PREC_TF32X3) {
-    L.hf_rh = c.take<float>(BN * H);
     L.hf_do32 = c.take<float>(BN * 32);
     L.hf_split = c.take<float>(max(gemm_nt_scratch_floats(HEAD_HID, (int)H), gemm_nt_scratch_floats((int)H, HEAD_HID)));
-    L.hf_loss_floats = BN / 8 + 2;
+    L.hf_loss_floats = BN / 128 + 2;
     L.hf_loss = c.take<float>(L.hf_loss_floats);
   }
   L.a1 = c.take<float>(BN * HEAD_HID);
diff --git a/regt-gcn_b200/csrc/common.cuh b/regt-gcn_b200/csrc/common.cuh
--- a/regt-gcn_b200/csrc/common.cuh
+++ b/regt-gcn_b200/csrc/common.cuh
@@ -115,7 +115,6 @@
   float* d_a1;
   float* D;
   float* Feat;
-  float* hf_rh;
   float* hf_do32;
   float* hf_split;
   float* hf_loss;
diff --git a/regt-gcn_b200/csrc/gemm_nt_ts.cuh b/regt-gcn_b200/csrc/gemm_nt_ts.cuh
--- /dev/null
+++ b/regt-gcn_b200/csrc/gemm_nt_ts.cuh
@@ -0,0 +1,221 @@
+#pragma once
+#include <cuda.h>
+
+#include "cell_tc.cuh"
+
+namespace regt {
+
+constexpr int NT_KC = 32;
+constexpr int NT_TILE = 128 * 128;
+constexpr int NT_MAXS = 6;
+constexpr int NT_SMEM_BUDGET = 227 * 1024 - 1024;
+
+__device__ __forceinline__ uint32_t tf32_rn(float a) {
+  uint32_t u;
+  asm("cvt.rna.tf32.f32 %0, %1;" : "=r"(u) : "f"(a));
+  return u;
+}
+__device__ __forceinline__ void split4(const float4 v, float4& hi, float4& lo) {
+  hi.x = __uint_as_float(tf32_rn(v.x)); hi.y = __uint_as_float(tf32_rn(v.y));
+  hi.z = __uint_as_float(tf32_rn(v.z)); hi.w = __uint_as_float(tf32_rn(v.w));
+  lo.x = v.x - hi.x; lo.y = v.y - hi.y; lo.z = v.z - hi.z; lo.w = v.w - hi.w;
+}
+__device__ __forceinline__ void tma_2d(void* dst, const CUtensorMap* map, int c0, int c1, uint64_t* bar) {
+  asm volatile(
+      "cp.async.bulk.tensor.2d.shared::cluster.global.tile.mbarrier::complete_tx::bytes [%0], [%1, {%2, %3}], [%4];" ::"r"(
+          tc::smem_u32(dst)),
+      "l"(reinterpret_cast<uint64_t>(map)), "r"(c0), "r"(c1), "r"(tc::smem_u32(bar))
+      : "memory");
+}
+__device__ __forceinline__ void tmap_prefetch(const CUtensorMap* map) {
+  asm volatile("prefetch.tensormap [%0];" ::"l"(reinterpret_cast<uint64_t>(map)) : "memory");
+}
+
+struct NtArgs {
+  CUtensorMap ta, tbh, tbl;
+  long long M;
+  int N, K;
+  int resident;
+  int ns;
+};
+constexpr int NT_CONV = 256;
+constexpr int NT_W_TMA = NT_CONV / 32;
+constexpr int NT_W_MMA = NT_W_TMA + 1;
+constexpr int NT_W_EPI = NT_W_MMA + 1;
+constexpr int NT_THREADS = (NT_W_EPI + 4) * 32;
+
+int prepare_gemm_nt_tma(NtArgs* a, size_t* smem, int* grid, const float* A, long long lda, const float* Bt, long long ldb, long long M,
+                        int N, int K, float* scratch, cudaStream_t st);
+
+constexpr int TS_SLOTS = 4;
+template <class Epi>
+__global__ void __launch_bounds__(NT_THREADS, 1) k_gemm_nt_tma_ts(const __grid_constant__ NtArgs a, const __grid_constant__ Epi epi) {
+  using namespace tc;
+  extern __shared__ __align__(1024) uint8_t smem_raw[];
+  uint8_t* sm = smem_raw + ((1024u - (smem_u32(smem_raw) & 1023u)) & 1023u);
+  __shared__ uint64_t bar_tma[NT_MAXS], bar_rfree[NT_MAXS], bar_afull[TS_SLOTS], bar_afree[TS_SLOTS], bar_b, bar_acc_full[2], bar_acc_free[2];
+  __shared__ uint32_t tmem_base_s;
+  const int tid = threadIdx.x, warp = tid >> 5, lane = tid & 31;
+  const int ns = a.ns;
+  const int nchunks = (a.K + NT_KC - 1) / NT_KC;
+  const int ntn = (a.N + 127) / 128;
+  const long long ntiles = ((a.M + 127) / 128) * ntn;
+  const int stage_bytes = a.resident ? NT_TILE : 3 * NT_TILE;
+  uint8_t* bres = sm;
+  uint8_t* stages = sm + (a.resident ? nchunks * 2 * NT_TILE : 0);
+  if (tid == 0) {
+    for (int s = 0; s < ns; ++s) {
+      mbar_init(&bar_tma[s], 1);
+      mbar_init(&bar_rfree[s], a.resident ? NT_CONV : NT_CONV + 1);
+    }
+    for (int s = 0; s < TS_SLOTS; ++s) {
+      mbar_init(&bar_afull[s], NT_CONV);
+      mbar_init(&bar_afree[s], 1);
+    }
+    mbar_init(&bar_b, 1);
+    for (int b = 0; b < 2; ++b) {
+      mbar_init(&bar_acc_full[b], 1);
+      mbar_init(&bar_acc_free[b], 128);
+    }
+    fence_barrier_init();
+  }
+  if (warp == NT_W_MMA) tmem_alloc(&tmem_base_s, 512);
+  tc_fence_before();
+  __syncthreads();
+  tc_fence_after();
+  const uint32_t tmem = tmem_base_s;
+  const uint32_t tmem_a = tmem + 256;
+
+  if (warp < NT_W_TMA) {
+    const int q = warp & 3, half = warp >> 2;
+    const int r = q * 32 + lane;
+    const uint32_t tl = tmem_a + ((uint32_t)(q * 32) << 16) + 16 * half;
+    long long gc = 0;
+    for (long long tile = blockIdx.x; tile < ntiles; tile += gridDim.x) {
+      for (int kc = 0; kc < nchunks; ++kc, ++gc) {
+        const int s = (int)(gc % ns), sl = (int)(gc % TS_SLOTS);
+        mbar_wait(&bar_tma[s], (uint32_t)((gc / ns) & 1));
+        const uint8_t* rw = stages + (size_t)s * stage_bytes + r * 128;
+        uint32_t hi[16], lo[16];
+#pragma unroll
+        for (int c = 0; c < 4; ++c) {
+          float4 v = *reinterpret_cast<const float4*>(rw + (((half * 4 + c) ^ (r & 7)) << 4));
+          if (Epi::relu_a) v = make_float4(fmaxf(v.x, 0.f), fmaxf(v.y, 0.f), fmaxf(v.z, 0.f), fmaxf(v.w, 0.f));
+          float4 h, l;
+          split4(v, h, l);
+          hi[4 * c] = __float_as_uint(h.x); hi[4 * c + 1] = __float_as_uint(h.y); hi[4 * c + 2] = __float_as_uint(h.z); hi[4 * c + 3] = __float_as_uint(h.w);
+          lo[4 * c] = __float_as_uint(l.x); lo[4 * c + 1] = __float_as_uint(l.y); lo[4 * c + 2] = __float_as_uint(l.z); lo[4 * c + 3] = __float_as_uint(l.w);
+        }
+        if ((hi[0] | hi[4] | hi[8] | hi[12]) == 0x7FC0DEADu) __nanosleep(1);
+        mbar_arrive(&bar_rfree[s]);
+        if (gc >= TS_SLOTS) {
+          mbar_wait(&bar_afree[sl], (uint32_t)((gc / TS_SLOTS - 1) & 1));
+          tc_fence_after();
+        }
+        tmem_st16(tl + 64 * sl, hi);
+        tmem_st16(tl + 64 * sl + 32, lo);
+        tmem_st_wait();
+        tc_fence_before();
+        mbar_arrive(&bar_afull[sl]);
+      }
+    }
+  } else if (warp == NT_W_TMA) {
+    if (lane == 0) {
+      tmap_prefetch(&a.ta);
+      tmap_prefetch(&a.tbh);
+      tmap_prefetch(&a.tbl);
+      if (a.resident) {
+        mbar_arrive_expect_tx(&bar_b, (uint32_t)(nchunks * 2 * NT_TILE));
+        for (int kc = 0; kc < nchunks; ++kc) {
+          tma_2d(bres + (size_t)kc * 2 * NT_TILE, &a.tbh, kc * NT_KC, 0, &bar_b);
+          tma_2d(bres + (size_t)kc * 2 * NT_TILE + NT_TILE, &a.tbl, kc * NT_KC, 0, &bar_b);
+        }
+      }
+      long long gc = 0;
+      for (long long tile = blockIdx.x; tile < ntiles; tile += gridDim.x) {
+        const int m0 = (int)((tile / ntn) * 128), n0 = (int)(tile % ntn) * 128;
+        for (int kc = 0; kc < nchunks; ++kc, ++gc) {
+          const int s = (int)(gc % ns);
+          if (gc >= ns) mbar_wait(&bar_rfree[s], (uint32_t)((gc / ns - 1) & 1));
+          uint8_t* st = stages + (size_t)s * stage_bytes;
+          mbar_arrive_expect_tx(&bar_tma[s], (uint32_t)stage_bytes);
+          tma_2d(st, &a.ta, kc * NT_KC, m0, &bar_tma[s]);
+          if (!a.resident) {
+            tma_2d(st + NT_TILE, &a.tbh, kc * NT_KC, n0, &bar_tma[s]);
+            tma_2d(st + 2 * NT_TILE, &a.tbl, kc * NT_KC, n0, &bar_tma[s]);
+          }
+        }
+      }
+    }
+  } else if (warp == NT_W_MMA) {
+    const uint32_t bres0 = smem_u32(bres), stage0 = smem_u32(stages);
+    if (a.resident) mbar_wait(&bar_b, 0);
+    long long gc = 0, li = 0;
+    for (long long tile = blockIdx.x; tile < ntiles; tile += gridDim.x, ++li) {
+      const int nt = min(128, a.N - (int)(tile % ntn) * 128);
+      const uint32_t idesc = make_idesc(FMT_TF32, 128, nt, 0, 0);
+      const int buf = (int)(li & 1);
+      if (li >= 2) {
+        mbar_wait(&bar_acc_free[buf], (uint32_t)((li / 2 - 1) & 1));
+        tc_fence_after();
+      }
+      for (int kc = 0; kc < nchunks; ++kc, ++gc) {
+        const int sl = (int)(gc % TS_SLOTS);
+        mbar_wait(&bar_afull[sl], (uint32_t)((gc / TS_SLOTS) & 1));
+        tc_fence_after();
+        if (lane == 0) {
+          const uint32_t ah = tmem_a + 64 * sl, al = ah + 32;
+          const int s = (int)(gc % ns);
+          const uint32_t bt = a.resident ? bres0 + kc * 2 * NT_TILE : stage0 + s * stage_bytes + NT_TILE;
+#pragma unroll
+          for (int p = 0; p < 3; ++p) {
+            const uint32_t ap = (p == 1) ? al : ah, bp = bt + (p == 2 ? NT_TILE : 0);
+#pragma unroll
+            for (int k = 0; k < NT_KC / 8; ++k)
+              umma_ts_tf32(tmem + buf * 128, ap + 8 * k, make_desc(bp + k * 32, 16, 1024, LAYOUT_SW128), idesc,
+                           (kc > 0 || p > 0 || k > 0) ? 1u : 0u);
+          }
+          umma_commit(&bar_afree[sl]);
+          if (!a.resident) umma_commit(&bar_rfree[s]);
+          if (kc + 1 == nchunks) umma_commit(&bar_acc_full[buf]);
+        }
+        __syncwarp();
+      }
+    }
+    tc_fence_before();
+  } else {
+    const int r = (warp & 3) * 32 + lane;
+    const uint32_t tlane = tmem + ((uint32_t)((warp & 3) * 32) << 16);
+    typename Epi::Acc acc{};
+    long long li = 0;
+    for (long long tile = blockIdx.x; tile < ntiles; tile += gridDim.x, ++li) {
+      const int buf = (int)(li & 1);
+      const int n0 = (int)(tile % ntn) * 128;
+      const long long row = (tile / ntn) * 128 + r;
+      mbar_wait(&bar_acc_full[buf], (uint32_t)((li / 2) & 1));
+      tc_fence_after();
+      epi.tile(acc, tlane + buf * 128, row, row < a.M, n0, min(128, a.N - n0));
+      tc_fence_before();
+      mbar_arrive(&bar_acc_free[buf]);
+    }
+    epi.finish(acc, r);
+  }
+  __syncthreads();
+  if (warp == NT_W_MMA) tmem_dealloc(tmem, 512);
+}
+
+template <class Epi>
+int launch_gemm_nt_ts(const float* A, long long lda, const float* Bt, long long ldb, long long M, int N, int K, float* scratch,
+                      const Epi& epi, const char* name, cudaStream_t st, int* grid = nullptr) {
+  NtArgs a{};
+  size_t smem = 0;
+  int g = 0;
+  if (prepare_gemm_nt_tma(&a, &smem, &g, A, lda, Bt, ldb, M, N, K, scratch, st)) return -1;
+  REGT_CUDA(cudaFuncSetAttribute(k_gemm_nt_tma_ts<Epi>, cudaFuncAttributeMaxDynamicSharedMemorySize, (int)smem));
+  k_gemm_nt_tma_ts<Epi><<<g, NT_THREADS, smem, st>>>(a, epi);
+  REGT_LAUNCHED(name, st);
+  if (grid) *grid = g;
+  return 0;
+}
+
+}
diff --git a/regt-gcn_b200/csrc/gemm_tma.cu b/regt-gcn_b200/csrc/gemm_tma.cu
--- a/regt-gcn_b200/csrc/gemm_tma.cu
+++ b/regt-gcn_b200/csrc/gemm_tma.cu
@@ -1,36 +1,14 @@
 #include <cuda.h>
 
-#include "cell_tc.cuh"
+#include "gemm_nt_ts.cuh"
 
 namespace regt {
 using namespace tc;
 
 namespace {
-constexpr int KC = 32;
-constexpr int TILE = 128 * 128;
-constexpr int MAXS = 6;
-constexpr int SMEM_BUDGET = 227 * 1024 - 1024;
-
-__device__ __forceinline__ uint32_t tf32_rn(float a) {
-  uint32_t u;
-  asm("cvt.rna.tf32.f32 %0, %1;" : "=r"(u) : "f"(a));
-  return u;
-}
-__device__ __forceinline__ void split4(const float4 v, float4& hi, float4& lo) {
-  hi.x = __uint_as_float(tf32_rn(v.x)); hi.y = __uint_as_float(tf32_rn(v.y));
-  hi.z = __uint_as_float(tf32_rn(v.z)); hi.w = __uint_as_float(tf32_rn(v.w));
-  lo.x = v.x - hi.x; lo.y = v.y - hi.y; lo.z = v.z - hi.z; lo.w = v.w - hi.w;
-}
-__device__ __forceinline__ void tma_2d(void* dst, const CUtensorMap* map, int c0, int c1, uint64_t* bar) {
-  asm volatile(
-      "cp.async.bulk.tensor.2d.shared::cluster.global.tile.mbarrier::complete_tx::bytes [%0], [%1, {%2, %3}], [%4];" ::"r"(
-          smem_u32(dst)),
-      "l"(reinterpret_cast<uint64_t>(map)), "r"(c0), "r"(c1), "r"(smem_u32(bar))
-      : "memory");
-}
-__device__ __forceinline__ void tmap_prefetch(const CUtensorMap* map) {
-  asm volatile("prefetch.tensormap [%0];" ::"l"(reinterpret_cast<uint64_t>(map)) : "memory");
-}
+constexpr int KC = NT_KC;
+constexpr int TILE = NT_TILE;
+constexpr int SMEM_BUDGET = NT_SMEM_BUDGET;
 
 typedef CUresult (*EncodeFn)(CUtensorMap*, CUtensorMapDataType, cuuint32_t, void*, const cuuint64_t*, const cuuint64_t*,
                              const cuuint32_t*, const cuuint32_t*, CUtensorMapInterleave, CUtensorMapSwizzle,
@@ -70,190 +48,33 @@
   lo[i] = v - h;
 }
 
-struct NtArgs {
-  CUtensorMap ta, tbh, tbl;
+struct NtStore {
+  static constexpr bool relu_a = false;
+  struct Acc {};
   float* C;
-  long long M, ldc;
-  int N, K;
-  int resident;
-  int ns;
+  long long ldc;
+  __device__ __forceinline__ void tile(Acc&, uint32_t t, long long row, bool ok, int n0, int nt) const {
+    float* cp = C + (ok ? row : 0) * ldc + n0;
+    for (int c0 = 0; c0 < nt; c0 += 32) {
+      float v[32];
+      if (c0 + 32 <= nt) {
+        tc::tmem_ld32(t + c0, v);
+      } else {
+        float u[16];
+        tc::tmem_ld16(t + c0, u);
+#pragma unroll
+        for (int j = 0; j < 16; ++j) v[j] = u[j];
+      }
+      if (ok) {
+        const int w = min(32, nt - c0);
+#pragma unroll
+        for (int j = 0; j < 32; j += 4)
+          if (j < w) *reinterpret_cast<float4*>(cp + c0 + j) = make_float4(v[j], v[j + 1], v[j + 2], v[j + 3]);
+      }
+    }
+  }
+  __device__ __forceinline__ void finish(Acc&, int) const {}
 };
-constexpr int NT_CONV = 256;
-constexpr int NT_W_TMA = NT_CONV / 32;
-constexpr int NT_W_MMA = NT_W_TMA + 1;
-constexpr int NT_W_EPI = NT_W_MMA + 1;
-constexpr int NT_THREADS = (NT_W_EPI + 4) * 32;
-
-constexpr int TS_SLOTS = 4;
-__global__ void __launch_bounds__(NT_THREADS, 1) k_gemm_nt_tma_ts(const __grid_constant__ NtArgs a) {
-  extern __shared__ __align__(1024) uint8_t smem_raw[];
-  uint8_t* sm = smem_raw + ((1024u - (smem_u32(smem_raw) & 1023u)) & 1023u);
-  __shared__ uint64_t bar_tma[MAXS], bar_rfree[MAXS], bar_afull[TS_SLOTS], bar_afree[TS_SLOTS], bar_b, bar_acc_full[2], bar_acc_free[2];
-  __shared__ uint32_t tmem_base_s;
-  const int tid = threadIdx.x, warp = tid >> 5, lane = tid & 31;
-  const int ns = a.ns;
-  const int nchunks = (a.K + KC - 1) / KC;
-  const int ntn = (a.N + 127) / 128;
-  const long long ntiles = ((a.M + 127) / 128) * ntn;
-  const int stage_bytes = a.resident ? TILE : 3 * TILE;
-  uint8_t* bres = sm;
-  uint8_t* stages = sm + (a.resident ? nchunks * 2 * TILE : 0);
-  if (tid == 0) {
-    for (int s = 0; s < ns; ++s) {
-      mbar_init(&bar_tma[s], 1);
-      mbar_init(&bar_rfree[s], a.resident ? NT_CONV : NT_CONV + 1);
-    }
-    for (int s = 0; s < TS_SLOTS; ++s) {
-      mbar_init(&bar_afull[s], NT_CONV);
-      mbar_init(&bar_afree[s], 1);
-    }
-    mbar_init(&bar_b, 1);
-    for (int b = 0; b < 2; ++b) {
-      mbar_init(&bar_acc_full[b], 1);
-      mbar_init(&bar_acc_free[b], 128);
-    }
-    fence_barrier_init();
-  }
-  if (warp == NT_W_MMA) tmem_alloc(&tmem_base_s, 512);
-  tc_fence_before();
-  __syncthreads();
-  tc_fence_after();
-  const uint32_t tmem = tmem_base_s;
-  const uint32_t tmem_a = tmem + 256;
-
-  if (warp < NT_W_TMA) {
-    const int q = warp & 3, half = warp >> 2;
-    const int r = q * 32 + lane;
-    const uint32_t tl = tmem_a + ((uint32_t)(q * 32) << 16) + 16 * half;
-    long long gc = 0;
-    for (long long tile = blockIdx.x; tile < ntiles; tile += gridDim.x) {
-      for (int kc = 0; kc < nchunks; ++kc, ++gc) {
-        const int s = (int)(gc % ns), sl = (int)(gc % TS_SLOTS);
-        mbar_wait(&bar_tma[s], (uint32_t)((gc / ns) & 1));
-        const uint8_t* rw = stages + (size_t)s * stage_bytes + r * 128;
-        uint32_t hi[16], lo[16];
-#pragma unroll
-        for (int c = 0; c < 4; ++c) {
-          const float4 v = *reinterpret_cast<const float4*>(rw + (((half * 4 + c) ^ (r & 7)) << 4));
-          float4 h, l;
-          split4(v, h, l);
-          hi[4 * c] = __float_as_uint(h.x); hi[4 * c + 1] = __float_as_uint(h.y); hi[4 * c + 2] = __float_as_uint(h.z); hi[4 * c + 3] = __float_as_uint(h.w);
-          lo[4 * c] = __float_as_uint(l.x); lo[4 * c + 1] = __float_as_uint(l.y); lo[4 * c + 2] = __float_as_uint(l.z); lo[4 * c + 3] = __float_as_uint(l.w);
-        }
-        if ((hi[0] | hi[4] | hi[8] | hi[12]) == 0x7FC0DEADu) __nanosleep(1);
-        mbar_arrive(&bar_rfree[s]);
-        if (gc >= TS_SLOTS) {
-          mbar_wait(&bar_afree[sl], (uint32_t)((gc / TS_SLOTS - 1) & 1));
-          tc_fence_after();
-        }
-        tmem_st16(tl + 64 * sl, hi);
-        tmem_st16(tl + 64 * sl + 32, lo);
-        tmem_st_wait();
-        tc_fence_before();
-        mbar_arrive(&bar_afull[sl]);
-      }
-    }
-  } else if (warp == NT_W_TMA) {
-    if (lane == 0) {
-      tmap_prefetch(&a.ta);
-      tmap_prefetch(&a.tbh);
-      tmap_prefetch(&a.tbl);
-      if (a.resident) {
-        mbar_arrive_expect_tx(&bar_b, (uint32_t)(nchunks * 2 * TILE));
-        for (int kc = 0; kc < nchunks; ++kc) {
-          tma_2d(bres + (size_t)kc * 2 * TILE, &a.tbh, kc * KC, 0, &bar_b);
-          tma_2d(bres + (size_t)kc * 2 * TILE + TILE, &a.tbl, kc * KC, 0, &bar_b);
-        }
-      }
-      long long gc = 0;
-      for (long long tile = blockIdx.x; tile < ntiles; tile += gridDim.x) {
-        const int m0 = (int)((tile / ntn) * 128), n0 = (int)(tile % ntn) * 128;
-        for (int kc = 0; kc < nchunks; ++kc, ++gc) {
-          const int s = (int)(gc % ns);
-          if (gc >= ns) mbar_wait(&bar_rfree[s], (uint32_t)((gc / ns - 1) & 1));
-          uint8_t* st = stages + (size_t)s * stage_bytes;
-          mbar_arrive_expect_tx(&bar_tma[s], (uint32_t)stage_bytes);
-          tma_2d(st, &a.ta, kc * KC, m0, &bar_tma[s]);
-          if (!a.resident) {
-            tma_2d(st + TILE, &a.tbh, kc * KC, n0, &bar_tma[s]);
-            tma_2d(st + 2 * TILE, &a.tbl, kc * KC, n0, &bar_tma[s]);
-          }
-        }
-      }
-    }
-  } else if (warp == NT_W_MMA) {
-    const uint32_t bres0 = smem_u32(bres), stage0 = smem_u32(stages);
-    if (a.resident) mbar_wait(&bar_b, 0);
-    long long gc = 0, li = 0;
-    for (long long tile = blockIdx.x; tile < ntiles; tile += gridDim.x, ++li) {
-      const int nt = min(128, a.N - (int)(tile % ntn) * 128);
-      const uint32_t idesc = make_idesc(FMT_TF32, 128, nt, 0, 0);
-      const int buf = (int)(li & 1);
-      if (li >= 2) {
-        mbar_wait(&bar_acc_free[buf], (uint32_t)((li / 2 - 1) & 1));
-        tc_fence_after();
-      }
-      for (int kc = 0; kc < nchunks; ++kc, ++gc) {
-        const int sl = (int)(gc % TS_SLOTS);
-        mbar_wait(&bar_afull[sl], (uint32_t)((gc / TS_SLOTS) & 1));
-        tc_fence_after();
-        if (lane == 0) {
-          const uint32_t ah = tmem_a + 64 * sl, al = ah + 32;
-          const int s = (int)(gc % ns);
-          const uint32_t bt = a.resident ? bres0 + kc * 2 * TILE : stage0 + s * stage_bytes + TILE;
-#pragma unroll
-          for (int p = 0; p < 3; ++p) {
-            const uint32_t ap = (p == 1) ? al : ah, bp = bt + (p == 2 ? TILE : 0);
-#pragma unroll
-            for (int k = 0; k < KC / 8; ++k)
-              umma_ts_tf32(tmem + buf * 128, ap + 8 * k, make_desc(bp + k * 32, 16, 1024, LAYOUT_SW128), idesc,
-                           (kc > 0 || p > 0 || k > 0) ? 1u : 0u);
-          }
-          umma_commit(&bar_afree[sl]);
-          if (!a.resident) umma_commit(&bar_rfree[s]);
-          if (kc + 1 == nchunks) umma_commit(&bar_acc_full[buf]);
-        }
-        __syncwarp();
-      }
-    }
-    tc_fence_before();
-  } else {
-    const int r = (warp & 3) * 32 + lane;
-    const uint32_t tlane = tmem + ((uint32_t)((warp & 3) * 32) << 16);
-    long long li = 0;
-    for (long long tile = blockIdx.x; tile < ntiles; tile += gridDim.x, ++li) {
-      const int buf = (int)(li & 1);
-      const int n0 = (int)(tile % ntn) * 128;
-      const int nt = min(128, a.N - n0);
-      const long long arow = (tile / ntn) * 128 + r;
-      const bool a_ok = arow < a.M;
-      float* cp = a.C + (a_ok ? arow : 0) * a.ldc + n0;
-      mbar_wait(&bar_acc_full[buf], (uint32_t)((li / 2) & 1));
-      tc_fence_after();
-      for (int c0 = 0; c0 < nt; c0 += 32) {
-        float v[32];
-        if (c0 + 32 <= nt) {
-          tmem_ld32(tlane + buf * 128 + c0, v);
-        } else {
-          float u[16];
-          tmem_ld16(tlane + buf * 128 + c0, u);
-#pragma unroll
-          for (int j = 0; j < 16; ++j) v[j] = u[j];
-        }
-        if (a_ok) {
-          const int w = min(32, nt - c0);
-#pragma unroll
-          for (int j = 0; j < 32; j += 4)
-            if (j < w) *reinterpret_cast<float4*>(cp + c0 + j) = make_float4(v[j], v[j + 1], v[j + 2], v[j + 3]);
-        }
-      }
-      tc_fence_before();
-      mbar_arrive(&bar_acc_free[buf]);
-    }
-  }
-  __syncthreads();
-  if (warp == NT_W_MMA) tmem_dealloc(tmem, 512);
-}
 
 struct TnSeg {
   int k0, k1;
@@ -676,31 +497,32 @@
 
 size_t gemm_nt_scratch_floats(int N, int K) { return (size_t)2 * ((N + 127) / 128 * 128) * ((K + KC - 1) / KC * KC); }
 
-int launch_gemm_nt_tma(const float* A, long long lda, const float* Bt, long long ldb, float* C, long long ldc, long long M, int N,
-                       int K, float* scratch, cudaStream_t st) {
-  REGT_CHECK(A && Bt && C && scratch && M >= 1 && N > 0 && N % 16 == 0 && K > 0 && K % 4 == 0 && ldc % 4 == 0 &&
-                 ((uintptr_t)C % 16) == 0 && ((uintptr_t)scratch % 16) == 0,
+int prepare_gemm_nt_tma(NtArgs* a, size_t* smem, int* grid, const float* A, long long lda, const float* Bt, long long ldb, long long M,
+                        int N, int K, float* scratch, cudaStream_t st) {
+  REGT_CHECK(A && Bt && scratch && M >= 1 && N > 0 && N % 16 == 0 && K > 0 && K % 4 == 0 && ((uintptr_t)scratch % 16) == 0,
              "gemm_nt_tma: bad operands (M=%lld N=%d K=%d)", M, N, K);
   const int Np = (N + 127) / 128 * 128, Kp = (K + KC - 1) / KC * KC, nchunks = Kp / KC;
   float* hi = scratch;
   float* lo = scratch + (size_t)Np * Kp;
   k_split_hilo<<<cdiv((long long)Np * Kp, 256), 256, 0, st>>>(Bt, ldb, N, K, Np, Kp, hi, lo);
   REGT_LAUNCHED("k_split_hilo", st);
-  NtArgs a{};
-  if (tmap_2d(&a.ta, A, K, M, lda, 128, "gemm_nt_tma(A)")) return -1;
-  if (tmap_2d(&a.tbh, hi, Kp, Np, Kp, 128, "gemm_nt_tma(B hi)")) return -1;
-  if (tmap_2d(&a.tbl, lo, Kp, Np, Kp, 128, "gemm_nt_tma(B lo)")) return -1;
-  a.C = C; a.M = M; a.ldc = ldc; a.N = N; a.K = K;
-  a.resident = (N <= 128 && nchunks * 2 * TILE + 2 * 2 * TILE <= SMEM_BUDGET) ? 1 : 0;
-  const int fixed = a.resident ? nchunks * 2 * TILE : 0;
-  const int stage_ts = a.resident ? TILE : 3 * TILE;
-  a.ns = min(MAXS, (SMEM_BUDGET - fixed) / stage_ts);
-  const long long ntiles = (long long)cdiv(M, 128) * cdiv(N, 128);
-  const size_t smem_ts = (size_t)fixed + (size_t)a.ns * stage_ts + 1024;
-  REGT_CUDA(cudaFuncSetAttribute(k_gemm_nt_tma_ts, cudaFuncAttributeMaxDynamicSharedMemorySize, (int)smem_ts));
-  k_gemm_nt_tma_ts<<<(int)min(ntiles, (long long)sm_count()), NT_THREADS, smem_ts, st>>>(a);
-  REGT_LAUNCHED("k_gemm_nt_tma_ts", st);
+  if (tmap_2d(&a->ta, A, K, M, lda, 128, "gemm_nt_tma(A)")) return -1;
+  if (tmap_2d(&a->tbh, hi, Kp, Np, Kp, 128, "gemm_nt_tma(B hi)")) return -1;
+  if (tmap_2d(&a->tbl, lo, Kp, Np, Kp, 128, "gemm_nt_tma(B lo)")) return -1;
+  a->M = M; a->N = N; a->K = K;
+  a->resident = (N <= 128 && nchunks * 2 * TILE + 2 * 2 * TILE <= SMEM_BUDGET) ? 1 : 0;
+  const int fixed = a->resident ? nchunks * 2 * TILE : 0;
+  const int stage_ts = a->resident ? TILE : 3 * TILE;
+  a->ns = min(NT_MAXS, (SMEM_BUDGET - fixed) / stage_ts);
+  *smem = (size_t)fixed + (size_t)a->ns * stage_ts + 1024;
+  *grid = (int)min((long long)cdiv(M, 128) * cdiv(N, 128), (long long)sm_count());
   return 0;
+}
+
+int launch_gemm_nt_tma(const float* A, long long lda, const float* Bt, long long ldb, float* C, long long ldc, long long M, int N,
+                       int K, float* scratch, cudaStream_t st) {
+  REGT_CHECK(C && ldc % 4 == 0 && ((uintptr_t)C % 16) == 0, "gemm_nt_tma: bad output");
+  return launch_gemm_nt_ts(A, lda, Bt, ldb, M, N, K, scratch, NtStore{C, ldc}, "k_gemm_nt_tma_ts", st);
 }
 
 int launch_gemm_tn_tma(const float* A, long long lda, long long M, int Ktot, int nseg, const int* seg_k0, const int* seg_b,
diff --git a/regt-gcn_b200/csrc/head_f.cu b/regt-gcn_b200/csrc/head_f.cu
--- a/regt-gcn_b200/csrc/head_f.cu
+++ b/regt-gcn_b200/csrc/head_f.cu
@@ -1,96 +1,105 @@
-#include "common.cuh"
+#include "gemm_nt_ts.cuh"
 
 namespace regt {
 
 namespace {
-__global__ void __launch_bounds__(256) k_hf_relu(const float4* __restrict__ hid, float4* __restrict__ rh, long long n4) {
-  const long long i = blockIdx.x * (long long)blockDim.x + threadIdx.x;
-  if (i >= n4) return;
-  const float4 v = __ldg(hid + i);
-  rh[i] = make_float4(fmaxf(v.x, 0.f), fmaxf(v.y, 0.f), fmaxf(v.z, 0.f), fmaxf(v.w, 0.f));
-}
-
 constexpr int HF_O = 16;
-__global__ void __launch_bounds__(256) k_hf_mid(float* __restrict__ a1, const float* __restrict__ b1, const float* __restrict__ w2,
-                                                const float* __restrict__ b2, const float* __restrict__ y, long long BN, int O, float scale,
-                                                float* __restrict__ out, float* __restrict__ d_out, float* __restrict__ loss_part) {
-  __shared__ float red[8];
-  const int lane = threadIdx.x & 31, warp = threadIdx.x >> 5;
-  float w[HF_O][4];
-#pragma unroll
-  for (int o = 0; o < HF_O; ++o) {
-    const float4 t = o < O ? __ldg(reinterpret_cast<const float4*>(w2 + (size_t)o * HEAD_HID) + lane) : make_float4(0.f, 0.f, 0.f, 0.f);
-    w[o][0] = t.x; w[o][1] = t.y; w[o][2] = t.z; w[o][3] = t.w;
-  }
-  const float4 bb = __ldg(reinterpret_cast<const float4*>(b1) + lane);
-  float lsum = 0.f;
-  for (long long q = blockIdx.x * 8ll + warp; q < BN; q += (long long)gridDim.x * 8) {
-    const float4 p = reinterpret_cast<const float4*>(a1 + q * HEAD_HID)[lane];
-    const float a[4] = {fmaxf(p.x + bb.x, 0.f), fmaxf(p.y + bb.y, 0.f), fmaxf(p.z + bb.z, 0.f), fmaxf(p.w + bb.w, 0.f)};
-    reinterpret_cast<float4*>(a1 + q * HEAD_HID)[lane] = make_float4(a[0], a[1], a[2], a[3]);
-    float s16[HF_O];
-#pragma unroll
-    for (int o = 0; o < HF_O; ++o) {
-      float s = a[0] * w[o][0];
-      s = fmaf(a[1], w[o][1], s); s = fmaf(a[2], w[o][2], s); s = fmaf(a[3], w[o][3], s);
-      s16[o] = s;
-    }
-    float s8[8], s4[4], s2[2];
-    {
-      const bool up = lane & 16;
-#pragma unroll
-      for (int i = 0; i < 8; ++i) {
-        const float keep = up ? s16[i + 8] : s16[i], send = up ? s16[i] : s16[i + 8];
-        s8[i] = keep + __shfl_xor_sync(0xffffffffu, send, 16);
+
+constexpr int HF_W2 = 0, HF_B1 = HF_O * HEAD_HID, HF_B2 = HF_B1 + HEAD_HID, HF_PACK = HF_B2 + HF_O;
+struct HeadMidArgs {
+  const float* wp;
+  const float* y;
+  float *a1, *out, *d_out;
+  float* loss_part;
+  int O;
+  float scale;
+};
+template <int NO>
+struct HeadMid : HeadMidArgs {
+  static constexpr bool relu_a = true;
+  struct Acc {
+    float lsum;
+  };
+  static constexpr int CW = NO > 8 ? 8 : 16;
+
+  __device__ __forceinline__ void tile(Acc& acc, uint32_t t, long long q, bool ok, int, int) const {
+    float s[NO];
+#pragma unroll
+    for (int o = 0; o < NO; ++o) s[o] = 0.f;
+    float* a1r = a1 + (ok ? q : 0) * HEAD_HID;
+#pragma unroll 1
+    for (int c0 = 0; c0 < HEAD_HID; c0 += CW) {
+      float v[CW];
+      tc::tmem_ld<CW>(t + c0, v);
+#pragma unroll
+      for (int j = 0; j < CW; j += 4) {
+        const float4 bb = __ldg(reinterpret_cast<const float4*>(wp + HF_B1 + c0 + j));
+        v[j] = fmaxf(v[j] + bb.x, 0.f); v[j + 1] = fmaxf(v[j + 1] + bb.y, 0.f);
+        v[j + 2] = fmaxf(v[j + 2] + bb.z, 0.f); v[j + 3] = fmaxf(v[j + 3] + bb.w, 0.f);
+#pragma unroll
+        for (int o = 0; o < NO; ++o) {
+          const float4 w = __ldg(reinterpret_cast<const float4*>(wp + HF_W2 + o * HEAD_HID + c0 + j));
+          s[o] = fmaf(v[j], w.x, s[o]); s[o] = fmaf(v[j + 1], w.y, s[o]);
+          s[o] = fmaf(v[j + 2], w.z, s[o]); s[o] = fmaf(v[j + 3], w.w, s[o]);
+        }
+        if (ok) *reinterpret_cast<float4*>(a1r + c0 + j) = make_float4(v[j], v[j + 1], v[j + 2], v[j + 3]);
       }
     }
-    {
-      const bool up = lane & 8;
-#pragma unroll
-      for (int i = 0; i < 4; ++i) {
-        const float keep = up ? s8[i + 4] : s8[i], send = up ? s8[i] : s8[i + 4];
-        s4[i] = keep + __shfl_xor_sync(0xffffffffu, send, 8);
+#pragma unroll
+    for (int o = 0; o < NO; ++o) {
+      if (ok && o < O) {
+        const float v = s[o] + __ldg(wp + HF_B2 + o);
+        out[q * O + o] = v;
+        if (y) {
+          const float diff = v - __ldg(y + q * O + o);
+          acc.lsum = fmaf(diff, diff, acc.lsum);
+          d_out[q * O + o] = 2.0f * diff * scale;
+        }
       }
     }
-    {
-      const bool up = lane & 4;
-#pragma unroll
-      for (int i = 0; i < 2; ++i) {
-        const float keep = up ? s4[i + 2] : s4[i], send = up ? s4[i] : s4[i + 2];
-        s2[i] = keep + __shfl_xor_sync(0xffffffffu, send, 4);
+  }
+
+  __device__ __forceinline__ void finish(Acc& acc, int r) const {
+    if (!y) return;
+    __shared__ float red[4];
+    float s = acc.lsum;
+#pragma unroll
+    for (int d = 16; d > 0; d >>= 1) s += __shfl_xor_sync(0xffffffffu, s, d);
+    if ((r & 31) == 0) red[r >> 5] = s;
+    asm volatile("bar.sync 1, 128;" ::: "memory");
+    if (r == 0) loss_part[blockIdx.x] = (red[0] + red[1] + red[2] + red[3]) * scale;
+  }
+};
+
+struct HeadGmask {
+  static constexpr bool relu_a = false;
+  struct Acc {};
+  const float* hid;
+  const float* dh;
+  float* G;
+  int H, tiled;
+
+  __device__ __forceinline__ void tile(Acc&, uint32_t t, long long q, bool ok, int n0, int nt) const {
+    const float* hr = hid + (ok ? q : 0) * H + n0;
+    const float* dr = dh ? dh + (ok ? q : 0) * H + n0 : nullptr;
+    for (int c0 = 0; c0 < nt; c0 += 32) {
+      float v[32];
+      tc::tmem_ld32(t + c0, v);
+      if (!ok) continue;
+#pragma unroll
+      for (int j = 0; j < 32; j += 4) {
+        const float4 h = __ldg(reinterpret_cast<const float4*>(hr + c0 + j));
+        float4 g = make_float4(h.x > 0.f ? v[j] : 0.f, h.y > 0.f ? v[j + 1] : 0.f, h.z > 0.f ? v[j + 2] : 0.f, h.w > 0.f ? v[j + 3] : 0.f);
+        if (dr) {
+          const float4 e = __ldg(reinterpret_cast<const float4*>(dr + c0 + j));
+          g.x += e.x; g.y += e.y; g.z += e.z; g.w += e.w;
+        }
+        *reinterpret_cast<float4*>(G + g_off(q, n0 + c0 + j, H, tiled)) = g;
       }
     }
-    float mine;
-    {
-      const bool up = lane & 2;
-      const float keep = up ? s2[1] : s2[0], send = up ? s2[0] : s2[1];
-      mine = keep + __shfl_xor_sync(0xffffffffu, send, 2);
-    }
-    mine += __shfl_xor_sync(0xffffffffu, mine, 1);
-    const int o = lane >> 1;
-    if ((lane & 1) == 0 && o < O) {
-      const float v = mine + __ldg(b2 + o);
-      out[q * O + o] = v;
-      if (y) {
-        const float diff = v - __ldg(y + q * O + o);
-        lsum = fmaf(diff, diff, lsum);
-        d_out[q * O + o] = 2.0f * diff * scale;
-      }
-    }
-  }
-  if (y) {
-#pragma unroll
-    for (int d = 16; d > 0; d >>= 1) lsum += __shfl_xor_sync(0xffffffffu, lsum, d);
-    if (lane == 0) red[warp] = lsum;
-    __syncthreads();
-    if (threadIdx.x == 0) {
-      float s = 0.f;
-#pragma unroll
-      for (int i = 0; i < 8; ++i) s += red[i];
-      loss_part[blockIdx.x] = s * scale;
-    }
-  }
-}
+  }
+  __device__ __forceinline__ void finish(Acc&, int) const {}
+};
 
 __global__ void __launch_bounds__(256) k_hf_da1(const float* __restrict__ a1, const float* __restrict__ w2, const float* __restrict__ d_out,
                                                 long long BN, int O, float* __restrict__ d_a1, float* __restrict__ dO32) {
@@ -113,21 +122,14 @@
   dO32[q * 32 + lane] = lane < O ? dv : (lane == 16 ? 1.0f : 0.f);
 }
 
-__global__ void __launch_bounds__(256) k_hf_gmask(const float4* __restrict__ gpre, const float4* __restrict__ hid, const float4* __restrict__ dh,
-                                                  long long BN, int H, int tiled, float* __restrict__ G) {
-  const long long i = blockIdx.x * (long long)blockDim.x + threadIdx.x;
-  const int h4 = H >> 2;
-  if (i >= BN * h4) return;
-  const long long q = i / h4;
-  const int n = (int)(i - q * h4) * 4;
-  const float4 g = __ldg(gpre + i), h = __ldg(hid + i);
-  float4 v = make_float4(h.x > 0.f ? g.x : 0.f, h.y > 0.f ? g.y : 0.f, h.z > 0.f ? g.z : 0.f, h.w > 0.f ? g.w : 0.f);
-  if (dh) {
-    const float4 d = __ldg(dh + i);
-    v.x += d.x; v.y += d.y; v.z += d.z; v.w += d.w;
-  }
-  *reinterpret_cast<float4*>(G + g_off(q, n, H, tiled)) = v;
-}
+__global__ void k_hf_pack(const float* __restrict__ w2, const float* __restrict__ b1, const float* __restrict__ b2, int O,
+                          float* __restrict__ wp) {
+  const int i = blockIdx.x * blockDim.x + threadIdx.x;
+  if (i < HF_B1) wp[i] = i / HEAD_HID < O ? w2[i] : 0.f;
+  else if (i < HF_B2) wp[i] = b1[i - HF_B1];
+  else if (i < HF_PACK) wp[i] = i - HF_B2 < O ? b2[i - HF_B2] : 0.f;
+}
+
 __global__ void k_hf_w1t(const float* __restrict__ w1, int H, float* __restrict__ W1t) {
   const int i = blockIdx.x * blockDim.x + threadIdx.x;
   if (i >= H * HEAD_HID) return;
@@ -142,24 +144,39 @@
   for (int z = 0; z < splits; ++z) s += C2[((size_t)z * HEAD_HID + n) * 32 + o];
   dW2[i] = acc ? dW2[i] + s : s;
 }
+
+template <int NO>
+int launch_head_mid(const regt_args* a, const Layout& L, const HeadMidArgs& p, cudaStream_t st, int* grid) {
+  HeadMid<NO> e;
+  static_cast<HeadMidArgs&>(e) = p;
+  return launch_gemm_nt_ts(a->out_hidden, a->H, a->p.head_w1, a->H, (long long)a->B * a->N, HEAD_HID, a->H, L.hf_split, e, "k_hf_mid",
+                           st, grid);
+}
 }
 
 bool head_f_fits(int O) { return O <= HF_O; }
 
 int head_forward_f(const regt_args* a, const Layout& L, cudaStream_t st) {
-  const int H = a->H, O = a->O;
-  const long long BN = (long long)a->B * a->N;
+  const int O = a->O;
   const int Nl = a->loss_nodes > 0 ? a->loss_nodes : a->N;
-  k_hf_relu<<<cdiv(BN * H / 4, 256), 256, 0, st>>>(reinterpret_cast<const float4*>(a->out_hidden), reinterpret_cast<float4*>(L.hf_rh), BN * H / 4);
-  REGT_LAUNCHED("k_hf_relu", st);
-  if (launch_gemm_nt_tma(L.hf_rh, H, a->p.head_w1, H, L.a1, HEAD_HID, BN, HEAD_HID, H, L.hf_split, st)) return -1;
-  const int nblk = (int)min((long long)cdiv(BN, 8), 1184ll);
   REGT_CHECK(!a->y || (a->loss && a->d_out), "head_forward: y given but loss/d_out is NULL");
-  REGT_CHECK(!a->y || (size_t)nblk <= L.hf_loss_floats, "head_forward: loss partial buffer too small");
-  k_hf_mid<<<nblk, 256, 0, st>>>(L.a1, a->p.head_b1, a->p.head_w2, a->p.head_b2, a->y, BN, O, 1.0f / ((float)Nl * (float)O), a->out,
-                                 a->d_out, L.hf_loss);
-  REGT_LAUNCHED("k_hf_mid", st);
-  if (a->y) return launch_reduce_splits(L.hf_loss, a->loss, 1, nblk, 0, st);
+  float* wp = L.part;
+  k_hf_pack<<<cdiv(HF_PACK, 256), 256, 0, st>>>(a->p.head_w2, a->p.head_b1, a->p.head_b2, O, wp);
+  REGT_LAUNCHED("k_hf_pack", st);
+  HeadMidArgs e{};
+  e.wp = wp; e.y = a->y;
+  e.a1 = L.a1; e.out = a->out; e.d_out = a->d_out;
+  e.loss_part = L.hf_loss; e.O = O; e.scale = 1.0f / ((float)Nl * (float)O);
+  int grid = 0, rc;
+  switch ((O + 3) / 4) {
+    case 1: rc = launch_head_mid<4>(a, L, e, st, &grid); break;
+    case 2: rc = launch_head_mid<8>(a, L, e, st, &grid); break;
+    case 3: rc = launch_head_mid<12>(a, L, e, st, &grid); break;
+    default: rc = launch_head_mid<16>(a, L, e, st, &grid); break;
+  }
+  if (rc) return rc;
+  REGT_CHECK((size_t)grid <= L.hf_loss_floats, "head_forward: loss partial buffer too small");
+  if (a->y) return launch_reduce_splits(L.hf_loss, a->loss, 1, grid, 0, st);
   return 0;
 }
 
@@ -171,10 +188,8 @@
   float* W1t = L.part + L.part_floats - (size_t)H * HEAD_HID;
   k_hf_w1t<<<cdiv((long long)H * HEAD_HID, 256), 256, 0, st>>>(a->p.head_w1, H, W1t);
   REGT_LAUNCHED("k_hf_w1t", st);
-  if (launch_gemm_nt_tma(L.d_a1, HEAD_HID, W1t, HEAD_HID, L.hf_rh, H, BN, H, HEAD_HID, L.hf_split, st)) return -1;
-  k_hf_gmask<<<cdiv(BN * (H / 4), 256), 256, 0, st>>>(reinterpret_cast<const float4*>(L.hf_rh), reinterpret_cast<const float4*>(a->out_hidden),
-                                                      reinterpret_cast<const float4*>(a->d_hidden), BN, H, L.route.g_tiled, L.G);
-  REGT_LAUNCHED("k_hf_gmask", st);
+  const HeadGmask g{a->out_hidden, a->d_hidden, L.G, H, L.route.g_tiled ? 1 : 0};
+  if (launch_gemm_nt_ts(L.d_a1, HEAD_HID, W1t, HEAD_HID, BN, H, HEAD_HID, L.hf_split, g, "k_hf_gmask", st)) return -1;
   float* part = L.part;
   if (launch_head_dw1_tf32x3(a, L, L.hf_do32, st)) return -1;
   const int s2 = (int)max(1ll, min(148ll, BN / 256));
```

Result: no change. 232.4 (median of 6 runs) (+1.0%).
